# mmetcalf14/qml-cutensornet

Hardware: AMD Instinct MI355X
Metric: Gram kernel entries/sec @ 60 qubits x 6 layers (higher is better)
Workload: dtype f64 (complex128)

## Files before the change

include/qkgram.h:

```cpp
#ifndef QKGRAM_H
#define QKGRAM_H

#include <stdint.h>

#ifdef __cplusplus
extern "C" {
#endif

#define QK_OK 0
#define QK_EINVAL (-1)
#define QK_EDEVICE (-2)
#define QK_ENOMEM (-3)

#define QK_LAYOUT_LPR 0
#define QK_LAYOUT_LRP 1

#define QK_PLAN_SYMMETRIC 1u
#define QK_PLAN_QUADS 2u

#define QK_PLAN_ORIENT 4u

typedef struct qk_ctx qk_ctx;
typedef struct qk_mps_set qk_mps_set;
typedef struct qk_plan qk_plan;

typedef struct qk_stats {
  int64_t pairs;
  double flops;
  double padded_flops;
  double bytes;
  double kernel_ms;
  int32_t grid;
  int32_t max_bond;
  int32_t kernel;
  int32_t precision;
  int64_t second_pairs;
  double second_flops, second_padded_flops, second_bytes;
  double second_ms;
  int32_t second_kernel;
  int32_t queues;
  double tail_frac, second_tail_frac;
  double derive_ms;
} qk_stats;

#define QK_KERNEL_NONE 0
#define QK_KERNEL_WAVE 1
#define QK_KERNEL_SMALL 2
#define QK_KERNEL_FUSED1 3
#define QK_KERNEL_FUSED2 4
#define QK_KERNEL_RING 5
#define QK_KERNEL_LAB 6
#define QK_KERNEL_WAVE2 7
#define QK_KERNEL_WAVE2_PLAIN 9
#define QK_KERNEL_FUSED_DUAL 8
#define QK_KERNEL_FUSED_DUAL_DET 10
#define QK_KERNEL_FUSED2_DET 11
#define QK_KERNEL_FUSED1_DET 12
const char* qk_kernel_name(int32_t kernel, int32_t precision);

const char* qk_last_error(void);

int qk_device_count(void);

int qk_ctx_create(int device_id, qk_ctx** out);
int qk_ctx_destroy(qk_ctx* ctx);
int qk_ctx_set_stream(qk_ctx* ctx, void* hip_stream);
int qk_ctx_use_own_stream(qk_ctx* ctx);
int qk_ctx_synchronize(qk_ctx* ctx);
int qk_ctx_trim(qk_ctx* ctx);

int qk_mps_set_create(qk_ctx* ctx, int32_t n_states, int32_t n_sites, const int32_t* bond_dims,
                      const double* const* site_tensors, int32_t layout, qk_mps_set** out);
int qk_mps_set_destroy(qk_mps_set* set);
int qk_mps_set_info(const qk_mps_set* set, int32_t* n_states, int32_t* n_sites, int32_t* max_padded_bond,
                    int64_t* device_bytes);

int qk_mps_set_image(const qk_mps_set* set, int64_t* n_doubles, const double** planes_dev, int32_t* dims_true, int64_t* offsets);
int qk_mps_set_copy_image(const qk_mps_set* set, double* dst, int64_t n_doubles);
int qk_mps_set_from_packed(qk_ctx* ctx, int32_t n_states, int32_t n_sites, const int32_t* dims_true, const int64_t* offsets,
                           const double* planes_dev, int64_t n_doubles, qk_mps_set** out);

int qk_mps_set_precision(const qk_mps_set* set);
int qk_mps_set_to_f32(qk_ctx* ctx, const qk_mps_set* src, qk_mps_set** out);

int64_t qk_pack_state_size(int32_t n_sites, const int32_t* bond_dims);
int qk_pack_state(int32_t n_sites, const int32_t* bond_dims, const double* const* site_tensors, int32_t layout,
                  double* out, int64_t* site_offsets );

int qk_plan_create(int32_t n_sites, int32_t nx, const int32_t* x_dims, int32_t ny, const int32_t* y_dims,
                   uint32_t flags, int32_t world_size, int32_t rank, int32_t block, qk_plan** out);
int qk_plan_destroy(qk_plan* plan);
int64_t qk_plan_num_pairs(const qk_plan* plan);
int64_t qk_plan_total_pairs(const qk_plan* plan);
int64_t qk_plan_max_pairs_per_rank(const qk_plan* plan);
const int32_t* qk_plan_pairs(const qk_plan* plan);
int qk_plan_stats(const qk_plan* plan, qk_stats* out);
int64_t qk_plan_first_run(const qk_plan* plan);
int qk_plan_queues(const qk_plan* plan, int64_t* qstart );
int32_t qk_plan_edge_sites(const qk_plan* plan);
int qk_plan_create_all(int32_t n_sites, int32_t nx, const int32_t* x_dims, int32_t ny, const int32_t* y_dims,
                       uint32_t flags, int32_t world_size, qk_plan** out);
int qk_plan_cost(const qk_plan* plan, double* plan_ms, int32_t* threads, double* tile_reuse_bytes);

int qk_gram_values(qk_ctx* ctx, const qk_mps_set* xset, const qk_mps_set* yset, const qk_plan* plan,
                   double* values_dev, double* z_dev);

int qk_gram_values_host(qk_ctx* ctx, const qk_mps_set* xset, const qk_mps_set* yset, const qk_plan* plan,
                        double* values_host, double* z_host);

int qk_scatter(qk_ctx* ctx, const int32_t* pairs_dev, const double* values_dev, int64_t n, double* k_dev,
               int64_t ld, int32_t mirror);

int qk_gram_host(qk_ctx* ctx, const qk_mps_set* xset, const qk_mps_set* yset, double* out, int64_t ld);

int qk_overlaps_host(qk_ctx* ctx, const qk_mps_set* xset, const qk_mps_set* yset, double* out);

int qk_get_stats(qk_ctx* ctx, qk_stats* out);

int qk_local_paulis_host(qk_ctx* ctx, const qk_mps_set* set, double* out ,
                         double* norms );

int qk_projected_gram_host(qk_ctx* ctx, int32_t n_sites, int32_t nx, const double* fx ,
                           int32_t ny, const double* fy , double g, double* out, int64_t ld);

int qk_local_pair_paulis_host(qk_ctx* ctx, const qk_mps_set* set, double* out2 ,
// ... 172 lines not shown
```

lab/qk_quad.h:

```cpp
#pragma once

__device__ __forceinline__ int qkq_qinv(const int d) {
  static constexpr int T[17] = {0, 1048576, 524288, 349526, 262144, 209716, 174763, 149797, 131072, 116509, 104858, 95326, 87382, 80660, 74899, 69906, 65536};
  return T[d];
}

struct QkqUnit {
  bool mine, a1, b1;
  int ta, tb, p;
};

template <bool A1, bool B1, typename XPtr>
__device__ __forceinline__ void qkq_p1(QkfTile (&T)[2][2], v2d (&fr)[4], v2d (&fs)[4], const bool primed, QkfStream cur, XPtr xp, unsigned x0, unsigned x1, const int nks,
                                       const QkfStream n0, const unsigned n1off) {
  v4d P[2][2][3];
  v2d fx[4], fy[4];
  if (!primed) qkf_load4(fr, cur);
  if (B1) {
#pragma unroll
    for (int i = 0; i < 4; ++i) fs[i] = qkf_ldg(cur.base + i * cur.step, cur.off + TILE);
  }
#pragma unroll
  for (int i = 0; i < 4; ++i) {
    fx[i] = qkf_ldx(xp + i * QKF_XSTEP, x0);
// ... 91 lines not shown
      if (FULL || i < kmax) {
        const double sp = fs[i].x + fs[i].y, sm = fs[i].x - fs[i].y;
        p1 = __builtin_amdgcn_mfma_f64_16x16x4f64(S[1][0][i], fs[i].x, p1, 0, 0, 0);
        p2 = __builtin_amdgcn_mfma_f64_16x16x4f64(T[1][0].re[i], sp, p2, 0, 0, 0);
        p3 = __builtin_amdgcn_mfma_f64_16x16x4f64(T[1][0].im[i], sm, p3, 0, 0, 0);
        if (B1) {
          r1 = __builtin_amdgcn_mfma_f64_16x16x4f64(S[1][1][i], fs[i].x, r1, 0, 0, 0);
          r2 = __builtin_amdgcn_mfma_f64_16x16x4f64(T[1][1].re[i], sp, r2, 0, 0, 0);
          r3 = __builtin_amdgcn_mfma_f64_16x16x4f64(T[1][1].im[i], sm, r3, 0, 0, 0);
        }
      }
      if (!LAST) fs[i] = qkf_ldg(i == 0 ? b0 : i == 1 ? b1 : i == 2 ? b2 : b3, o1);
      __builtin_amdgcn_sched_barrier(0);
    }
  }
  QKF_PRIO_HI();
  {
    const v4d re = p1 - p3, im = p1 - p2;
#pragma unroll
    for (int r = 0; r < 4; ++r) {
      __hip_atomic_fetch_add(d + r * rs, re[r], __ATOMIC_RELAXED, __HIP_MEMORY_SCOPE_WORKGROUP);
      __hip_atomic_fetch_add(d + r * rs + 1, im[r], __ATOMIC_RELAXED, __HIP_MEMORY_SCOPE_WORKGROUP);
    }
  }
  if (B1) {
    const v4d re = r1 - r3, im = r1 - r2;
#pragma unroll
    for (int r = 0; r < 4; ++r) {
      __hip_atomic_fetch_add(d1 + r * rs, re[r], __ATOMIC_RELAXED, __HIP_MEMORY_SCOPE_WORKGROUP);
      __hip_atomic_fetch_add(d1 + r * rs + 1, im[r], __ATOMIC_RELAXED, __HIP_MEMORY_SCOPE_WORKGROUP);
    }
  }
}

template <bool FULL, bool A1, bool B1>
__device__ __forceinline__ void qkq_p2(const QkfTile (&T)[2][2], v2d (&fr)[4], v2d (&fs)[4], const QkfStream cur, const unsigned a1off, const int ps, const int nn, const int kmax, lds_v2d* xo,
                                       const int q, const int j, const QkfStream nxt) {
  lds_double* d = (lds_double*)(xo + q * TILE + j);
  lds_double* d1 = d + 2 * QKF_XBLOCK;
  constexpr long rs = 2 * QKF_XSTEP;
  v4d S[2][2];
#pragma unroll
  for (int u = 0; u < 2; ++u)
#pragma unroll
    for (int v = 0; v < 2; ++v) S[u][v] = ((u == 0 || A1) && (v == 0 || B1)) ? T[u][v].re + T[u][v].im : (v4d){0, 0, 0, 0};
  const v2d *const c0 = cur.base, *const c1 = cur.base + cur.step, *const c2 = cur.base + 2 * cur.step, *const c3 = cur.base + 3 * cur.step;
  unsigned o0 = cur.off, o1 = cur.off + a1off;
#pragma unroll 1
  for (int tn = 0; tn + 1 < nn; ++tn) {
    o0 += TILE, o1 += TILE;
    qkq_p2_block<FULL, A1, B1, false>(T, S, fr, fs, kmax, c0, c1, c2, c3, o0, o1, d, d1, rs);
    d += 2 * ps, d1 += 2 * ps;
  }
  qkq_p2_block<FULL, A1, B1, true>(T, S, fr, fs, kmax, nxt.base, nxt.base + nxt.step, nxt.base + 2 * nxt.step, nxt.base + 3 * nxt.step, nxt.off, 0u, d, d1, rs);
}

template <int NW, int XCAP, int WPS>
__global__ __launch_bounds__(64 * NW, WPS) void qk_sweep_fused_quad_kernel(const SweepArgs g) {
  constexpr int NT = 64 * NW;
  extern __shared__ __attribute__((aligned(16))) double lds_raw[];
  lds_v2d* const XL = (lds_v2d*)lds_raw;
  long long* const slot = reinterpret_cast<long long*>(lds_raw + 2 * XCAP);
  const v2d* const xdata = reinterpret_cast<const v2d*>(g.xdata);
  const v2d* const ydata = reinterpret_cast<const v2d*>(g.ydata);
  v2d* const G0 = reinterpret_cast<v2d*>(g.scratch) + (long long)blockIdx.x * 2 * g.x_plane;
  const int tid = threadIdx.x, lane = tid & 63;
  const int wave = __builtin_amdgcn_readfirstlane(tid >> 6);
  const int j = lane & 15, q = lane >> 4;
  const int ns = g.n_sites;
  __attribute__((address_space(3))) double* const zacc = (__attribute__((address_space(3))) double*)(slot + 2);
  lds_v4i* const rec = (lds_v4i*)(slot + 2 + 32);
  long long* const m_off = reinterpret_cast<long long*>(slot + 2 + 32) + 6 * (long long)ns;
  auto rfl = [&](const int v) __attribute__((always_inline)) { return __builtin_amdgcn_readfirstlane(v); };
  auto ldl = [&](const long long* p_) __attribute__((always_inline)) {
    const long long v = *p_;
    const unsigned lo = __builtin_amdgcn_readfirstlane((unsigned)v);
    const unsigned hi = __builtin_amdgcn_readfirstlane((unsigned)((unsigned long long)v >> 32));
    return (long long)(((unsigned long long)hi << 32) | lo);
  };
  auto site = [&](const int k) __attribute__((always_inline)) {
    const v4i r0 = rec[3 * k], r1 = rec[3 * k + 1], r2 = rec[3 * k + 2];
    QkfSite s;
    s.a = rfl(r0.x), s.a2 = rfl(r0.y), s.b = rfl(r0.z), s.b2 = rfl(r0.w);
    s.at = rfl(r1.x), s.nks = rfl(r1.y), s.W = rfl(r1.z), s.small = rfl(r1.w) != 0;
    s.inv = rfl(r2.x);
    s.ps = rfl(r2.y), s.pd = 1 << s.ps, s.next = rfl(r2.z);
    s.mt = s.a / TILE, s.nt = s.b2 / TILE, s.nn = s.a2 / TILE;
    s.Ak = xdata + ldl(m_off + 2 * k);
    s.Bk = ydata + ldl(m_off + 2 * k + 1);
    return s;
  };
  struct Pieces {
    int qa_f, qb_f, ra, rb, nA, kq, n2a, nB, nC, nD, L, qinv;
  };
  auto pieces_of = [&](const QkfSite& s, const int w) __attribute__((always_inline)) {
    Pieces pc;
    pc.qa_f = s.mt >> 1, pc.qb_f = w >> 1, pc.ra = s.mt & 1, pc.rb = w & 1;
    pc.nA = s.pd * pc.qa_f * pc.qb_f;
#if defined(QKF_QUAD_MODE) && QKF_QUAD_MODE == 0
    pc.kq = 0;
#else
    pc.kq = pc.nA - pc.nA % NW;
#endif
    pc.n2a = 2 * (pc.nA - pc.kq);
    pc.nB = s.pd * pc.ra * pc.qb_f, pc.nC = s.pd * pc.qa_f * pc.rb, pc.nD = s.pd * pc.ra * pc.rb;
    pc.L = pc.kq + pc.n2a + pc.nB + pc.nC + pc.nD;
    pc.qinv = qkq_qinv(pc.qa_f);
    return pc;
  };
  auto unit_of = [&](const QkfSite& s, const int w, const Pieces& pc, const int r0) __attribute__((always_inline)) {
    QkqUnit un;
    const int left = pc.L - r0;
    const bool cut = 2 * left <= NW;
    const int sub = cut && wave >= left ? 1 : 0;
    int i = r0 + wave - sub * left;
    un.mine = cut ? wave < 2 * left : i < pc.L;
    un.a1 = un.b1 = false, un.ta = un.tb = un.p = 0;
    auto quad = [&](const int vq) __attribute__((always_inline)) {
      const int u = vq >> s.ps, qb = (u * pc.qinv) >> 20, qa = u - qb * pc.qa_f;
      un.p = vq & (s.pd - 1), un.ta = 2 * qa, un.tb = 2 * qb;
    };
    if (i < pc.kq) {
      quad(i), un.a1 = un.b1 = true;
    } else if ((i -= pc.kq) < pc.n2a) {
      quad(pc.kq + (i >> 1)), un.ta += i & 1, un.b1 = true;
    } else if ((i -= pc.n2a) < pc.nB) {
      un.p = i & (s.pd - 1), un.ta = s.mt - 1, un.tb = 2 * (i >> s.ps), un.b1 = true;
    } else if ((i -= pc.nB) < pc.nC) {
      un.p = i & (s.pd - 1), un.ta = 2 * (i >> s.ps), un.tb = w - 1, un.a1 = true;
    } else {
      i -= pc.nC;
      un.p = i & (s.pd - 1), un.ta = s.mt - 1, un.tb = w - 1;
    }
    if (cut) {
      if (un.b1) un.tb += sub, un.b1 = false;
      else if (un.a1) un.ta += sub, un.a1 = false;
      else un.mine = un.mine && sub == 0;
    }
    return un;
  };
  auto b_stream = [&](const QkfSite& s, const int s0, const QkqUnit& un) __attribute__((always_inline)) {
    return QkfStream{s.Bk + un.p * s.b2, (unsigned)((q * s.pd) * s.b2 + (s0 + un.tb) * TILE + j), 4 * s.pd * s.b2};
  };
  auto a_stream = [&](const QkfSite& s, const QkqUnit& un) __attribute__((always_inline)) {
    return QkfStream{s.Ak + un.p * s.a2, (unsigned)(((un.ta * TILE + q) * s.pd) * s.a2 + j), 4 * s.pd * s.a2};
  };
  const int xcc = qk_xcc_id();
  if (tid == 0) qk_tail_start(g);
  for (;;) {
    if (tid == 0) *slot = qk_pull(g, xcc);
    __syncthreads();
    const long long p = *slot;
    __syncthreads();
    if (p < 0) break;
    const int xi = g.pairs[2 * p], yj = g.pairs[2 * p + 1];
    qkf_step_table<XCAP, NT>(g, xi, yj, p, rec, m_off, tid, QkSegRule{XCAP, NW, true});
    const int ek = g.edge_k, k_hi = ns - ek;
    const bool edges = ek > 0;
    if (!edges)
      for (int e = tid; e < TILE * TILE; e += NT) XL[e] = (v2d){e == 0 ? 1.0 : 0.0, 0.0};
    __syncthreads();
    bool xg = false;
    int cur = 0, xb = 0;
    if (edges) {
      const v4i r0 = rec[3 * ek];
      const int a_e = rfl(r0.x), b_e = rfl(r0.z);
      xg = a_e * b_e > XCAP;
// ... 135 lines not shown
```

qml-cutensornet_amd/csrc/qk_fused.h:

```cpp
#pragma once
#include "qk_device.h"
#include "qk_plan.h"

#define QKF_PRIO_LO() __builtin_amdgcn_s_setprio(0)
#define QKF_PRIO_HI() __builtin_amdgcn_s_setprio(2)
typedef double v2d __attribute__((ext_vector_type(2)));
typedef __attribute__((address_space(3))) v2d lds_v2d;
static constexpr int QKF_XSTEP = 4 * TILE;
static constexpr int QKF_XBLOCK = TILE * TILE;


#ifndef QKF_LDS3M
#define QKF_LDS3M 0
#endif
#ifndef QKF_P2_PROBE
#define QKF_P2_PROBE 0
#endif
#ifndef QKF_ABL
#define QKF_ABL 0
#endif
#define QKF_STEP_BARRIER()                            \
  do {                                                \
    if (QKF_ABL & 4) asm volatile("s_waitcnt lgkmcnt(0)" ::: "memory"); \
    else qk_lds_barrier();                            \
  } while (0)
#define QKF_SUM(a, b) ((QKF_ABL & 1) ? (a) : (a) + (b))
#define QKF_DIF(a, b) ((QKF_ABL & 1) ? (b) : (a) - (b))
template <bool CONJB>
__device__ __forceinline__ void qkf_kstep(v4d& p1, v4d& p2, v4d& p3, const double ar, const double ai, const double br, const double bi) {
  const double sa = QKF_SUM(ar, ai), sb = CONJB ? QKF_DIF(br, bi) : QKF_SUM(br, bi);
  p1 = __builtin_amdgcn_mfma_f64_16x16x4f64(ar, br, p1, 0, 0, 0);
  p2 = __builtin_amdgcn_mfma_f64_16x16x4f64(ai, bi, p2, 0, 0, 0);
  p3 = __builtin_amdgcn_mfma_f64_16x16x4f64(sa, sb, p3, 0, 0, 0);
}

struct QkfTile {
  v4d re, im;
};

__device__ __forceinline__ v2d qkf_ldg(const v2d* __restrict__ base, const unsigned off) {
  return *reinterpret_cast<const v2d*>(reinterpret_cast<const char*>(base) + (size_t)(off * 16u));
}
#ifndef QKF_NT_A
#define QKF_NT_A 0
#endif
#ifndef QKF_NT_B
#define QKF_NT_B 0
#endif
__device__ __forceinline__ v2d qkf_ldg_nt(const v2d* __restrict__ base, const unsigned off) {
  return __builtin_nontemporal_load(reinterpret_cast<const v2d*>(reinterpret_cast<const char*>(base) + (size_t)(off * 16u)));
}
__device__ __forceinline__ v2d qkf_ldg_a(const v2d* __restrict__ base, const unsigned off) { return QKF_NT_A ? qkf_ldg_nt(base, off) : qkf_ldg(base, off); }
__device__ __forceinline__ v2d qkf_ldg_b(const v2d* __restrict__ base, const unsigned off) { return QKF_NT_B ? qkf_ldg_nt(base, off) : qkf_ldg(base, off); }
__device__ __forceinline__ v2d qkf_ldx(const v2d* __restrict__ base, const unsigned off) { return qkf_ldg(base, off); }
__device__ __forceinline__ v2d qkf_ldx(const lds_v2d* base, const unsigned off) { return base[off]; }

struct QkfStream {
  const v2d* base;
  unsigned off;
  int step;
  int lim = 4;
};
__device__ __forceinline__ const v2d* qkf_kbase(const v2d* const base, const int step, const int i, const int lim) { return base + max(min(i, lim - 1), 0) * step; }
__device__ __forceinline__ void qkf_load4(v2d (&fr)[4], const QkfStream& st) {
#pragma unroll
  for (int i = 0; i < 4; ++i) fr[i] = qkf_ldg(qkf_kbase(st.base, st.step, i, st.lim), st.off);
}
__device__ __forceinline__ v2d qkf_ldgb(const v2d* __restrict__ base, const unsigned boff) {
  const v2d* const at = reinterpret_cast<const v2d*>(reinterpret_cast<const char*>(base) + (size_t)boff);
  return QKF_NT_B ? __builtin_nontemporal_load(at) : *at;
}
struct QkfXLds {
  const lds_v2d* p;
  __device__ __forceinline__ void advance() { p += 4 * QKF_XSTEP; }
  __device__ __forceinline__ v2d kstep(const int i) const { return p[i * QKF_XSTEP]; }
};
struct QkfXGlobal {
  const v2d* base;
  unsigned bo;
  __device__ __forceinline__ void advance() { bo += 4 * QKF_XSTEP * 16u; }
  __device__ __forceinline__ v2d kstep(const int i) const { return *reinterpret_cast<const v2d*>(reinterpret_cast<const char*>(base + i * QKF_XSTEP) + (size_t)bo); }
};
__device__ __forceinline__ QkfXLds qkf_xcursor(const lds_v2d* xp, const unsigned xoff) { return QkfXLds{xp + xoff}; }
__device__ __forceinline__ QkfXGlobal qkf_xcursor(const v2d* xp, const unsigned xoff) { return QkfXGlobal{xp, xoff * 16u}; }

// ... 420 lines not shown
  QKF_PRIO_HI();
  t0.re = acc[0] + acc[1], t0.im = acc[2] - acc[0] + acc[1];
  if (HAS1) t1.re = acc[3] + acc[4], t1.im = acc[5] - acc[3] + acc[4];
}
__device__ __forceinline__ long long qkf_uniform(const long long v) {
  const unsigned lo = __builtin_amdgcn_readfirstlane((unsigned)v);
  const unsigned hi = __builtin_amdgcn_readfirstlane((unsigned)((unsigned long long)v >> 32));
  return (long long)(((unsigned long long)hi << 32) | lo);
}

template <int NW, bool PAIRS>
__device__ __forceinline__ QkEdgeUnit qkf_edge_unit_of(const int u, const int mt, const int nt, const int inv) {
  if constexpr (PAIRS) return qk_edge_unit(u, mt, nt, NW, inv);
  const int tb = (u * inv) >> 20;
  return QkEdgeUnit{u - tb * mt, tb, false, true};
}
template <int NW, bool PAIRS, int SETS>
__device__ __forceinline__ void qkf_edge_prefix(const SweepArgs& g, const int xi, const int yj, const int a, const int b, lds_v2d* const xl, v2d* const xg, const bool to_global, const int wave,
                                                const int q, const int j, const bool swap = false) {
  const v2d* const Lx = reinterpret_cast<const v2d*>(swap ? g.yedge : g.xedge) + qkf_uniform((swap ? g.yedge_offs : g.xedge_offs)[2 * (long long)xi]);
  const v2d* const Ly = reinterpret_cast<const v2d*>(swap ? g.xedge : g.yedge) + qkf_uniform((swap ? g.xedge_offs : g.yedge_offs)[2 * (long long)yj]);
  const int mt = a / TILE, nt = b / TILE, ng = (1 << g.edge_k) >> 4, inv = qk_recip20(mt), units = PAIRS ? qk_edge_units(mt, nt, NW) : mt * nt;
  for (int u = wave; u < units; u += NW) {
    const QkEdgeUnit un = qkf_edge_unit_of<NW, PAIRS>(u, mt, nt, inv);
    if (!un.mine) continue;
    QkfTile T0, T1;
    const unsigned oy = (unsigned)(q * b + un.tb0 * TILE + j), ox = (unsigned)(q * a + un.ta * TILE + j);
    if (un.has1) qkf_edge_unit<true, 1>(T0, T1, Ly, oy, b, Lx, ox, a, ng);
    else qkf_edge_unit<false, SETS>(T0, T1, Ly, oy, b, Lx, ox, a, ng);
    const int at = un.ta * (b * TILE) + (un.tb0 * TILE + q) * TILE + j;
    if (to_global) {
#pragma unroll
      for (int r = 0; r < 4; ++r) xg[at + r * QKF_XSTEP] = (v2d){T0.re[r], T0.im[r]};
      if (un.has1) {
#pragma unroll
        for (int r = 0; r < 4; ++r) xg[at + QKF_XBLOCK + r * QKF_XSTEP] = (v2d){T1.re[r], T1.im[r]};
      }
    } else {
#pragma unroll
      for (int r = 0; r < 4; ++r) xl[at + r * QKF_XSTEP] = (v2d){T0.re[r], T0.im[r]};
      if (un.has1) {
#pragma unroll
        for (int r = 0; r < 4; ++r) xl[at + QKF_XBLOCK + r * QKF_XSTEP] = (v2d){T1.re[r], T1.im[r]};
      }
    }
  }
}

template <int NW, bool PAIRS, int SETS>
__device__ __forceinline__ void qkf_edge_suffix(const SweepArgs& g, const int xi, const int yj, const int a, const int b, const lds_v2d* const xl, const v2d* const xg, const bool from_global,
                                                __attribute__((address_space(3))) double* zacc, const int wave, const int q, const int j, const bool swap = false) {
  const v2d* const Rx = reinterpret_cast<const v2d*>(swap ? g.yedge : g.xedge) + qkf_uniform((swap ? g.yedge_offs : g.xedge_offs)[2 * (long long)xi + 1]);
  const v2d* const Ry = reinterpret_cast<const v2d*>(swap ? g.xedge : g.yedge) + qkf_uniform((swap ? g.xedge_offs : g.yedge_offs)[2 * (long long)yj + 1]);
  const int mt = a / TILE, nt = b / TILE, ng = (1 << g.edge_k) >> 4, inv = qk_recip20(mt), units = PAIRS ? qk_edge_units(mt, nt, NW) : mt * nt;
  double zr = 0, zi = 0;
  for (int u = wave; u < units; u += NW) {
    const QkEdgeUnit un = qkf_edge_unit_of<NW, PAIRS>(u, mt, nt, inv);
    if (!un.mine) continue;
    QkfTile T0, T1;
    const unsigned oy = (unsigned)(q * b + un.tb0 * TILE + j), ox = (unsigned)(q * a + un.ta * TILE + j);
    if (un.has1) qkf_edge_unit<true, 1>(T0, T1, Ry, oy, b, Rx, ox, a, ng);
    else qkf_edge_unit<false, SETS>(T0, T1, Ry, oy, b, Rx, ox, a, ng);
    const int at = un.ta * (b * TILE) + (un.tb0 * TILE + q) * TILE + j;
#pragma unroll
    for (int r = 0; r < 4; ++r) {
      const v2d x = from_global ? xg[at + r * QKF_XSTEP] : (v2d)xl[at + r * QKF_XSTEP];
      zr += x.x * T0.re[r] - x.y * T0.im[r], zi += x.x * T0.im[r] + x.y * T0.re[r];
    }
    if (un.has1) {
#pragma unroll
      for (int r = 0; r < 4; ++r) {
        const v2d x = from_global ? xg[at + QKF_XBLOCK + r * QKF_XSTEP] : (v2d)xl[at + QKF_XBLOCK + r * QKF_XSTEP];
        zr += x.x * T1.re[r] - x.y * T1.im[r], zi += x.x * T1.im[r] + x.y * T1.re[r];
      }
    }
  }
#pragma unroll
  for (int o = 32; o > 0; o >>= 1) zr += __shfl_xor(zr, o), zi += __shfl_xor(zi, o);
  if ((q | j) == 0) zacc[2 * wave] = zr, zacc[2 * wave + 1] = zi;
}

struct QkfSite {
  int a, a2, b, b2, at, nks, mt, nt, nn, W, inv, inv2, pd, ps, next;
  bool small, sw;
  const v2d *Ak, *Bk;
};
typedef int v4i __attribute__((ext_vector_type(4)));
typedef __attribute__((address_space(3))) v4i lds_v4i;

template <int XCAP, int NT, bool ITEM_RECIPS = false>
__device__ __forceinline__ void qkf_step_table(const SweepArgs& g, const int xi, const int yj, const long long pair, lds_v4i* const rec, long long* const m_off, const int tid, const QkSegRule rule) {
  const int ns = g.n_sites, n1 = ns + 1;
  const int32_t* const xd = g.xdims + (long long)xi * n1;
  const int32_t* const yd = g.ydims + (long long)yj * n1;
  const int32_t* const xt = g.xtrue + (long long)xi * n1;
  const int32_t* const yt = g.ytrue + (long long)yj * n1;
  const v2d* const xdata = reinterpret_cast<const v2d*>(g.xdata);
  const v2d* const ydata = reinterpret_cast<const v2d*>(g.ydata);
  auto put = [&](const int e, const int len, const int o, const bool sw, const v2d* const X, const v2d* const Y) __attribute__((always_inline)) {
    const QkStepRec r = qk_step_record(xd, xt, yd, yt, e, len, o, sw, rule, ITEM_RECIPS);
    rec[3 * e] = (v4i){r.w[0], r.w[1], r.w[2], r.w[3]};
    rec[3 * e + 1] = (v4i){r.w[4], r.w[5], r.w[6], r.w[7]};
    rec[3 * e + 2] = (v4i){r.w[8], r.w[9], r.w[10], r.w[11]};
    m_off[2 * e] = (long long)(((const char*)(o ? Y : X) - (const char*)xdata) / 16);
    m_off[2 * e + 1] = (long long)(((const char*)(o ? X : Y) - (const char*)ydata) / 16);
  };
  auto plain = [&](const int e, const int o, const bool sw) __attribute__((always_inline)) {
    put(e, 1, o, sw, xdata + (g.xoffs[(long long)xi * ns + e] >> 1), ydata + (g.yoffs[(long long)yj * ns + e] >> 1));
  };
  if (g.seg == nullptr) {
    for (int e = tid; e < ns; e += NT) plain(e, 0, false);
    return;
  }
  const int ek = g.edge_k, k_hi = ns - ek;
  const unsigned long long w0 = g.seg[4 * pair], w1 = g.seg[4 * pair + 1], o0 = g.seg[4 * pair + 2], o1 = g.seg[4 * pair + 3];
  for (int e = ek + tid; e < k_hi; e += NT) {
    const int i = e - ek;
    const bool merged = qk_seg_bit(w0, w1, i) && e + 1 < k_hi;
    const int len = merged ? 2 : 1, o = qk_seg_bit(o0, o1, i) ? 1 : 0;
    const bool sw = qk_seg_bit(o0, o1, i + len) != (o != 0);
    if (merged)
      put(e, 2, o, sw, reinterpret_cast<const v2d*>(g.xmg) + (g.xmg_offs[(long long)xi * g.merge_steps + i] >> 1),
          reinterpret_cast<const v2d*>(g.ymg) + (g.ymg_offs[(long long)yj * g.merge_steps + i] >> 1));
    else plain(e, o, sw);
  }
}

#ifdef QKF_PROF
#define QKF_PROF_DECL() \
  unsigned long long pf[8] = {0, 0, 0, 0, 0, 0, 0, 0}, pt = __builtin_amdgcn_s_memtime(); \
  const unsigned long long pt0 = pt
#define QKF_STAMP(i)                                              \
  do {                                                            \
    const unsigned long long now_ = __builtin_amdgcn_s_memtime(); \
    pf[i] += now_ - pt;                                           \
    pt = now_;                                                    \
  } while (0)
#define QKF_PROF_FLUSH()                                             \
  do {                                                               \
    if (lane == 0) {                                                 \
      pf[7] = __builtin_amdgcn_s_memtime() - pt0;                    \
      for (int i_ = 0; i_ < 8; ++i_) atomicAdd(g.prof + i_, pf[i_]); \
    }                                                                \
  } while (0)
#else
#define QKF_PROF_DECL()
#define QKF_STAMP(i)
#define QKF_PROF_FLUSH()
#endif

#define QKF_PULLER(NT) ((NT) - 64)
__device__ __forceinline__ void qkf_pull_next(const SweepArgs& g, const int xcc, int& gang_round, long long* const word) {
  const long long pp = qk_pull(g, xcc);
  qk_gang_sync(g, xcc, pp >= 0, gang_round);
  *word = pp;
}

template <int NW, int S, int XCAP, int WPS, bool DET = false>
__global__ __launch_bounds__(64 * NW, WPS) void qk_sweep_fused_kernel(const SweepArgs g) {
  constexpr int NT = 64 * NW;
  extern __shared__ __attribute__((aligned(16))) double lds_raw[];
  lds_v2d* const XL = (lds_v2d*)lds_raw;
  long long* const slot = reinterpret_cast<long long*>(lds_raw + 2 * XCAP);
  const v2d* const xdata = reinterpret_cast<const v2d*>(g.xdata);
  const v2d* const ydata = reinterpret_cast<const v2d*>(g.ydata);
  v2d* const G0 = reinterpret_cast<v2d*>(g.scratch) + (long long)blockIdx.x * 2 * g.x_plane;
  const int tid = threadIdx.x, lane = tid & 63;
  const int wave = __builtin_amdgcn_readfirstlane(tid >> 6);
  const int j = lane & 15, q = lane >> 4;
  const int ns = g.n_sites;
  __attribute__((address_space(3))) double* const zacc = (__attribute__((address_space(3))) double*)(slot + 2);
  lds_v4i* const rec = (lds_v4i*)(slot + 2 + 32);
  long long* const m_off = reinterpret_cast<long long*>(slot + 2 + 32) + 6 * (long long)ns;
  lds_int* const tbroken = (lds_int*)(m_off + 2 * (long long)ns);
  lds_int* const turn0 = tbroken + 2;
  auto rfl = [&](const int v) __attribute__((always_inline)) { return __builtin_amdgcn_readfirstlane(v); };
  auto ldl = [&](const long long* p_) __attribute__((always_inline)) {
    const long long v = *p_;
    const unsigned lo = __builtin_amdgcn_readfirstlane((unsigned)v);
    const unsigned hi = __builtin_amdgcn_readfirstlane((unsigned)((unsigned long long)v >> 32));
    return (long long)(((unsigned long long)hi << 32) | lo);
  };
  auto site = [&](const int k) __attribute__((always_inline)) {
    const v4i r0 = rec[3 * k], r1 = rec[3 * k + 1], r2 = rec[3 * k + 2];
    QkfSite s;
    s.a = rfl(r0.x), s.a2 = rfl(r0.y), s.b = rfl(r0.z), s.b2 = rfl(r0.w);
    s.at = rfl(r1.x), s.nks = rfl(r1.y), s.W = rfl(r1.z), s.small = (rfl(r1.w) & QK_REC_SMALL) != 0, s.sw = (rfl(r1.w) & QK_REC_SWITCH) != 0;
    s.inv = rfl(r2.x), s.inv2 = rfl(r2.w);
    s.ps = rfl(r2.y), s.pd = 1 << s.ps, s.next = rfl(r2.z);
    s.mt = s.a / TILE, s.nt = s.b2 / TILE, s.nn = s.a2 / TILE;
    s.Ak = xdata + ldl(m_off + 2 * k);
    s.Bk = ydata + ldl(m_off + 2 * k + 1);
    return s;
  };
  auto item_of = [&](const QkfSite& s, const int w, const int it) __attribute__((always_inline)) {
    return DET ? qk_unit_decode_ordered(it, s.ps, s.mt, s.inv) : qk_unit_decode(it, s.mt, w, s.inv, qk_unit_recip_of(s.inv2, w == s.W));
  };
  auto b_stream = [&](const QkfSite& s, const int s0, const int w, const int it) __attribute__((always_inline)) {
    const QkUnit un = item_of(s, w, it);
    return QkfStream{s.Bk + un.p * s.b2, (unsigned)((q * s.pd) * s.b2 + (s0 + un.tc) * TILE + j), 4 * s.pd * s.b2, min(4, s.nks)};
  };
  auto a_stream = [&](const QkfSite& s, const int w, const int it) __attribute__((always_inline)) {
    const QkUnit un = item_of(s, w, it);
    return QkfStream{s.Ak + un.p * s.a2, (unsigned)(((un.ta * TILE + q) * s.pd) * s.a2 + j), 4 * s.pd * s.a2, min(4, (s.at - un.ta * TILE + 3) >> 2)};
  };
  QKF_PROF_DECL();
  const int xcc = qk_xcc_id();
  int gang_round = 0;
  if (tid == 0) qk_tail_start(g);
  for (;;) {
    if (tid == 0) {
      const long long pp_ = qk_pull(g, xcc);
      qk_gang_sync(g, xcc, pp_ >= 0, gang_round);
      *slot = pp_;
    }
    __syncthreads();
    const long long p = *slot;
    __syncthreads();
    if (p < 0) break;
    const int xi = g.pairs[2 * p], yj = g.pairs[2 * p + 1];
    qkf_step_table<XCAP, NT, true>(g, xi, yj, p, rec, m_off, tid, QkSegRule{XCAP, NW * S, false});
    const int ek = g.edge_k, k_hi = ns - ek;
    const bool edges = ek > 0;
    if (!edges)
      for (int e = tid; e < TILE * TILE; e += NT) XL[e] = (v2d){e == 0 ? 1.0 : 0.0, 0.0};
    if constexpr (DET)
      for (int e = tid; e < 2 * g.turn_ints + 2; e += NT) tbroken[e] = 0;
    int tsel = 0;
    __syncthreads();
    bool xg = false;
    int cur = 0, xb = 0;
    if (edges) {
      const v4i r0 = rec[3 * ek];
      const int a_e = rfl(r0.x), b_e = rfl(r0.z);
      const bool o1 = !DET && (rfl(rec[3 * ek + 1].w) & QK_REC_ORIENT) != 0;
      xg = a_e * b_e > XCAP;
      qkf_edge_prefix<NW, QKF_EDGE_PAIRS(WPS), QKF_EDGE_SETS(WPS)>(g, o1 ? yj : xi, o1 ? xi : yj, a_e, b_e, XL, G0, xg, wave, q, j, o1);
      __syncthreads();
    }
    QKF_STAMP(0);
    QkfTile T[S];
    v2d fr[4];
    bool primed = false;
    QkfSite sn = site(ek);
    for (int k = ek; k < k_hi;) {
      const QkfSite sc = sn;
      k = sc.next;
      if (k < k_hi) sn = site(k);
      const int a = sc.a, a2 = sc.a2, b = sc.b, mt = sc.mt, nt = sc.nt, W = sc.W;
      const bool small = sc.small;
      v2d* const Gc = G0 + (long long)cur * g.x_plane;
      v2d* const Gn = G0 + (long long)(cur ^ 1) * g.x_plane;
      if (small && xg) {
        for (int e = tid; e < a * b; e += NT) XL[e] = Gc[e];
        __syncthreads();
        xg = false, xb = 0;
      } else if (!small && !xg) {
        for (int e = tid; e < a * b; e += NT) Gc[e] = XL[xb + e];
        __syncthreads();
        xg = true;
      }
      const int n_out = sc.b2 * a2;
      const bool pingpong = small && a * b + n_out <= XCAP;
      const int ob = !small ? 0 : pingpong ? (xb == 0 ? XCAP - n_out : 0) : 0;
      if (pingpong && !DET)
        for (int e = tid; e < n_out; e += NT) XL[ob + e] = (v2d){0.0, 0.0};
      QKF_STAMP(1);
      for (int s0 = 0; s0 < nt; s0 += W) {
        const int w = min(W, nt - s0), items = sc.pd * mt * w;
        lds_int* const tcur = turn0 + tsel * g.turn_ints;
        if constexpr (DET) {
          for (int e = tid; e < g.turn_ints; e += NT) turn0[(tsel ^ 1) * g.turn_ints + e] = 0;
        } else if (!small) {
          for (int e = tid; e < w * TILE * a2; e += NT) XL[e] = (v2d){0.0, 0.0};
          QKF_STEP_BARRIER();
        }
        QKF_STAMP(6);
        for (int r0 = 0; r0 < items; r0 += NW * S) {
          const int L = min(S, (items - r0 + NW - 1) / NW);
          const bool multi = L > 1;
          const int it0 = r0 + wave;
          auto phase1 = [&](auto xbase) __attribute__((always_inline)) {
#pragma unroll 1
            for (int s = 0; s < L; ++s) {
              if (multi) qkf_rotate<S>(T, L);
              const int it = it0 + NW * s;
              if (it < items) {
                const int ta = item_of(sc, w, it).ta;
                const bool more = s + 1 < L && it + NW < items;
                const QkfStream nxt = more ? b_stream(sc, s0, w, it + NW) : a_stream(sc, w, it0);
                qkf_p1_tile(T[S - 1], fr, primed, b_stream(sc, s0, w, it), xbase, (unsigned)(ta * (b * TILE) + q * TILE + j), sc.nks, nxt);
                primed = true;
              }
            }
          };
          if (xg) phase1((const v2d*)Gc);
          else phase1((const lds_v2d*)(XL + xb));
          QKF_STAMP(2);
          if (small && r0 == 0 && !(DET && pingpong)) {
            QKF_STEP_BARRIER();
            if (!pingpong && !DET) {
              for (int e = tid; e < n_out; e += NT) XL[e] = (v2d){0.0, 0.0};
              QKF_STEP_BARRIER();
            }
          }
          QKF_STAMP(3);
          const bool last_round = s0 + W >= nt && r0 + NW * S >= items;
#pragma unroll 1
          for (int s = 0; s < S; ++s) {
            const int it = it0 + NW * s;
            if (it >= items) break;
            if (multi) qkf_rotate<S>(T, L);
            const QkUnit un = item_of(sc, w, it);
            const int ta = un.ta, tbl = un.tc;
            const int kmax = min(4, (sc.at - ta * TILE + 3) >> 2);
            const bool more = s + 1 < S && it + NW < items;
            const int wn = min(sn.W, sn.nt);
            const bool chain = !more && last_round && k < k_hi && wave < sn.pd * sn.mt * wn;
            const QkfStream nxt = more ? a_stream(sc, w, it + NW) : chain ? b_stream(sn, 0, wn, wave) : a_stream(sc, w, it);
            const int tix = sc.pd * ta + un.p;
            const QkfTurn turn{tcur + tbl * sc.nn, tix, tbroken, g.err};
            constexpr int FORM = DET ? 0 : WPS >= 4 ? QKF_P2_FORM_TWO : QKF_P2_FORM_ONE;
            if (!DET && sc.sw) {
              lds_double* const dsw = (lds_double*)(XL + ob + tbl * (a2 * TILE) + q * TILE + j);
              if (FORM != 0 && kmax == 4) qkf_p2_switch<true, false, FORM>(T[S - 1], T[S - 1], fr, primed, a_stream(sc, w, it), 4, sc.nn, 4, dsw, 0, nxt);
              else qkf_p2_switch<false, false, FORM>(T[S - 1], T[S - 1], fr, primed, a_stream(sc, w, it), kmax, sc.nn, kmax, dsw, 0, nxt);
            } else if (kmax == 4) qkf_p2_item<true, DET, FORM>(T[S - 1], fr, primed, a_stream(sc, w, it), w * QKF_XBLOCK, sc.nn, 4, XL + ob + tbl * QKF_XBLOCK, q, j, nxt, turn);
            else qkf_p2_item<false, DET, FORM>(T[S - 1], fr, primed, a_stream(sc, w, it), w * QKF_XBLOCK, sc.nn, kmax, XL + ob + tbl * QKF_XBLOCK, q, j, nxt, turn);
            primed = more || chain;
          }
          QKF_STAMP(4);
        }
        QKF_STEP_BARRIER();
        tsel ^= 1;
        QKF_STAMP(5);
        if (!small && nt > W) {
          for (int tn = 0; tn < sc.nn; ++tn)
            for (int e = tid; e < w * QKF_XBLOCK; e += NT) Gn[(long long)tn * (sc.b2 * TILE) + s0 * QKF_XBLOCK + e] = XL[tn * w * QKF_XBLOCK + e];
          __syncthreads();
          QKF_STAMP(1);
        }
      }
      if (!small) {
        if (nt > W) cur ^= 1;
        else xg = false, xb = 0;
      } else {
        xb = ob;
      }
    }
    const int fl_end = DET ? 0 : rfl(rec[3 * (k_hi - 1) + 1].w);
    const bool sw_end = (fl_end & QK_REC_SWITCH) != 0, o_end = ((fl_end & QK_REC_ORIENT) != 0) != sw_end;
    if (edges) {
      const v4i r0 = rec[3 * (k_hi - 1)];
      const int a_l = rfl(r0.y), b_l = rfl(r0.w), a_e = sw_end ? b_l : a_l, b_e = sw_end ? a_l : b_l;
      qkf_edge_suffix<NW, QKF_EDGE_PAIRS(WPS), QKF_EDGE_SETS(WPS)>(g, o_end ? yj : xi, o_end ? xi : yj, a_e, b_e, (const lds_v2d*)(XL + xb), (const v2d*)(G0 + (long long)cur * g.x_plane), xg, zacc, wave,
                                                                   q, j, o_end);
      __syncthreads();
    }
    if (tid == 0) {
      v2d zz = {0.0, 0.0};
      if (edges)
        for (int w_ = 0; w_ < NW; ++w_) zz.x += zacc[2 * w_], zz.y += zacc[2 * w_ + 1];
      else zz = xg ? G0[(long long)cur * g.x_plane] : (v2d)XL[xb];
      if (o_end) zz.y = -zz.y;
      g.values[p] = zz.x * zz.x + zz.y * zz.y;
      if (g.z) {
        g.z[2 * p] = zz.x;
        g.z[2 * p + 1] = zz.y;
      }
    }
    __syncthreads();
  }
  if (tid == 0) qk_tail_exit(g);
  QKF_PROF_FLUSH();
}

template <bool HAS1, typename XPtr>
__device__ __forceinline__ void qkf_p1_dual(QkfTile& t0, QkfTile& t1, v2d (&fr)[4], v2d (&fs)[4], const bool primed, QkfStream cur, XPtr xp, unsigned xoff, const int nks,
                                            const QkfStream nxt) {
  v4d p1 = {0, 0, 0, 0}, p2 = {0, 0, 0, 0}, p3 = {0, 0, 0, 0}, r1 = {0, 0, 0, 0}, r2 = {0, 0, 0, 0}, r3 = {0, 0, 0, 0};
  v2d fx[4];
  if (!primed) qkf_load4(fr, cur);
  if (HAS1) {
#pragma unroll
    for (int i = 0; i < 4; ++i) fs[i] = qkf_ldg(cur.base + i * cur.step, cur.off + TILE);
  }
#pragma unroll
  for (int i = 0; i < 4; ++i) fx[i] = qkf_ldx(xp + i * QKF_XSTEP, xoff);
  const int ng = (nks + 3) >> 2, last = nks - 4 * (ng - 1);
  QKF_PRIO_LO();
  int gq = 0;
  if (ng >= 2) {
    gq = 1;
    cur.off += 4 * cur.step, xoff += 4 * QKF_XSTEP;
#pragma unroll
    for (int i = 0; i < 4; ++i) {
      if (i == 0) {
        const v4d z = {0, 0, 0, 0};
        const double sa = QKF_SUM(fx[0].x, fx[0].y);
        p1 = __builtin_amdgcn_mfma_f64_16x16x4f64(fx[0].x, fr[0].x, z, 0, 0, 0);
        p2 = __builtin_amdgcn_mfma_f64_16x16x4f64(fx[0].y, fr[0].y, z, 0, 0, 0);
        p3 = __builtin_amdgcn_mfma_f64_16x16x4f64(sa, QKF_SUM(fr[0].x, fr[0].y), z, 0, 0, 0);
        if (HAS1) {
          r1 = __builtin_amdgcn_mfma_f64_16x16x4f64(fx[0].x, fs[0].x, z, 0, 0, 0);
          r2 = __builtin_amdgcn_mfma_f64_16x16x4f64(fx[0].y, fs[0].y, z, 0, 0, 0);
          r3 = __builtin_amdgcn_mfma_f64_16x16x4f64(sa, QKF_SUM(fs[0].x, fs[0].y), z, 0, 0, 0);
        }
      } else {
        qkf_kstep<false>(p1, p2, p3, fx[i].x, fx[i].y, fr[i].x, fr[i].y);
        if (HAS1) qkf_kstep<false>(r1, r2, r3, fx[i].x, fx[i].y, fs[i].x, fs[i].y);
      }
      if (!(QKF_ABL & 2)) fr[i] = qkf_ldg_b(cur.base + i * cur.step, cur.off);
      if (HAS1 && !(QKF_ABL & 2)) fs[i] = qkf_ldg_b(cur.base + i * cur.step, cur.off + TILE);
      if (!(QKF_ABL & 8)) fx[i] = qkf_ldx(xp + i * QKF_XSTEP, xoff);
      __builtin_amdgcn_sched_barrier(0);
    }
  }
#pragma unroll 1
  for (; gq + 1 < ng; ++gq) {
    cur.off += 4 * cur.step, xoff += 4 * QKF_XSTEP;
#pragma unroll
    for (int i = 0; i < 4; ++i) {
      qkf_kstep<false>(p1, p2, p3, fx[i].x, fx[i].y, fr[i].x, fr[i].y);
      if (HAS1) qkf_kstep<false>(r1, r2, r3, fx[i].x, fx[i].y, fs[i].x, fs[i].y);
      if (!(QKF_ABL & 2)) fr[i] = qkf_ldg_b(cur.base + i * cur.step, cur.off);
      if (HAS1 && !(QKF_ABL & 2)) fs[i] = qkf_ldg_b(cur.base + i * cur.step, cur.off + TILE);
      if (!(QKF_ABL & 8)) fx[i] = qkf_ldx(xp + i * QKF_XSTEP, xoff);
      __builtin_amdgcn_sched_barrier(0);
    }
  }
#pragma unroll
  for (int i = 0; i < 4; ++i) {
    if (i < last) {
      qkf_kstep<false>(p1, p2, p3, fx[i].x, fx[i].y, fr[i].x, fr[i].y);
      if (HAS1) qkf_kstep<false>(r1, r2, r3, fx[i].x, fx[i].y, fs[i].x, fs[i].y);
    }
    if (!(QKF_ABL & 2)) fr[i] = qkf_ldg(nxt.base + i * nxt.step, nxt.off);
    __builtin_amdgcn_sched_barrier(0);
  }
  QKF_PRIO_HI();
  t0.re = p1 - p2, t0.im = p3 - p1 - p2;
  if (HAS1) t1.re = r1 - r2, t1.im = r3 - r1 - r2;
}

template <bool FULL, bool HAS1>
__device__ __forceinline__ void qkf_p2_block(const QkfTile& t0, const QkfTile& t1, const v4d& s0, const v4d& s1, v2d (&fr)[4], const int kmax, const v2d* const b0, const v2d* const b1,
// ... 33 lines not shown
  if (HAS1) {
#pragma unroll
    for (int r = 0; r < 4; ++r) {
      __hip_atomic_fetch_add(d1 + r * rs, re1[r], __ATOMIC_RELAXED, __HIP_MEMORY_SCOPE_WORKGROUP);
      __hip_atomic_fetch_add(d1 + r * rs + 1, im1[r], __ATOMIC_RELAXED, __HIP_MEMORY_SCOPE_WORKGROUP);
    }
  }
}
template <bool FULL, bool HAS1, bool DET>
__device__ __forceinline__ void qkf_p2_dual_turn(const QkfTile& t0, const QkfTile& t1, v2d (&fr)[4], v2d (&fs)[4], QkfStream cur, const int ps, const int nn, const int kmax, lds_v2d* xo, const int q,
                                            const int j, const QkfStream nxt, const bool nxt_p1, const unsigned n1, const QkfTurn turn = QkfTurn{nullptr, 0, nullptr, nullptr}) {
  __attribute__((address_space(3))) double* d = (__attribute__((address_space(3))) double*)(xo + q * TILE + j);
#pragma unroll 1
  for (int tn = 0; tn < nn; ++tn) {
    v4d p1 = {0, 0, 0, 0}, p2 = {0, 0, 0, 0}, p3 = {0, 0, 0, 0}, r1 = {0, 0, 0, 0}, r2 = {0, 0, 0, 0}, r3 = {0, 0, 0, 0};
    const bool fin = tn + 1 == nn;
    const v2d* const rb = fin ? nxt.base : cur.base;
    const int rs = fin ? nxt.step : cur.step;
    cur.off = fin ? nxt.off : cur.off + TILE;
    QKF_PRIO_LO();
#pragma unroll
    for (int i = 0; i < 4; ++i) {
      if (FULL || i < kmax) {
        qkf_kstep<true>(p1, p2, p3, t0.re[i], t0.im[i], fr[i].x, fr[i].y);
        if (HAS1) qkf_kstep<true>(r1, r2, r3, t1.re[i], t1.im[i], fr[i].x, fr[i].y);
      }
      fr[i] = qkf_ldg_a(rb + i * rs, cur.off);
      __builtin_amdgcn_sched_barrier(0);
    }
    QKF_PRIO_HI();
    {
      const v4d re = p1 + p2, im = p3 - p1 + p2;
      if constexpr (DET) qkf_turn_add(d, (long)2 * QKF_XSTEP, re, im, turn, tn);
      else {
#pragma unroll
        for (int r = 0; r < 4; ++r) {
          __hip_atomic_fetch_add(d + r * 2 * QKF_XSTEP, re[r], __ATOMIC_RELAXED, __HIP_MEMORY_SCOPE_WORKGROUP);
          __hip_atomic_fetch_add(d + r * 2 * QKF_XSTEP + 1, im[r], __ATOMIC_RELAXED, __HIP_MEMORY_SCOPE_WORKGROUP);
        }
      }
    }
    if (HAS1) {
      const v4d re = r1 + r2, im = r3 - r1 + r2;
      __attribute__((address_space(3))) double* const d1 = d + 2 * QKF_XBLOCK;
      if constexpr (DET) qkf_turn_add(d1, (long)2 * QKF_XSTEP, re, im, QkfTurn{turn.at + nn, turn.idx, turn.broken, turn.gerr}, tn);
      else {
#pragma unroll
        for (int r = 0; r < 4; ++r) {
          __hip_atomic_fetch_add(d1 + r * 2 * QKF_XSTEP, re[r], __ATOMIC_RELAXED, __HIP_MEMORY_SCOPE_WORKGROUP);
          __hip_atomic_fetch_add(d1 + r * 2 * QKF_XSTEP + 1, im[r], __ATOMIC_RELAXED, __HIP_MEMORY_SCOPE_WORKGROUP);
        }
      }
    }
    d += 2 * ps;
  }
}

template <bool FULL, bool HAS1, bool DET = false>
__device__ __forceinline__ void qkf_p2_dual(const QkfTile& t0, const QkfTile& t1, v2d (&fr)[4], v2d (&fs)[4], QkfStream cur, const int ps, const int nn, const int kmax, lds_v2d* xo, const int q,
                                            const int j, const QkfStream nxt, const bool nxt_p1, const unsigned n1, const QkfTurn turn = QkfTurn{nullptr, 0, nullptr, nullptr}) {
  if constexpr (DET) {
    qkf_p2_dual_turn<FULL, HAS1, DET>(t0, t1, fr, fs, cur, ps, nn, kmax, xo, q, j, nxt, nxt_p1, n1, turn);
    return;
  }
  lds_double* d = (lds_double*)(xo + q * TILE + j);
  lds_double* d1 = d + 2 * QKF_XBLOCK;
  if constexpr (QKF_P2_FORM_DUAL != 0) {
    qkf_p2_blocks<FULL, HAS1, false>(t0, t1, fr, cur, 4, nxt, nn, kmax, d, 2 * QKF_XBLOCK, 2 * ps);
    return;
  }
  constexpr long rs = 2 * QKF_XSTEP;
  const v4d s0 = t0.re + t0.im, s1 = HAS1 ? t1.re + t1.im : s0;
  const v2d *const c0 = cur.base, *const c1 = cur.base + cur.step, *const c2 = cur.base + 2 * cur.step, *const c3 = cur.base + 3 * cur.step;
  unsigned off = cur.off;
#pragma unroll 1
  for (int tn = 0; tn + 1 < nn; ++tn) {
    off += TILE;
    qkf_p2_block<FULL, HAS1>(t0, t1, s0, s1, fr, kmax, c0, c1, c2, c3, off, d, d1, rs);
    d += 2 * ps, d1 += 2 * ps;
  }
  qkf_p2_block<FULL, HAS1>(t0, t1, s0, s1, fr, kmax, nxt.base, nxt.base + nxt.step, nxt.base + 2 * nxt.step, nxt.base + 3 * nxt.step, nxt.off, d, d1, rs);
}

template <int NW, int XCAP, int WPS, bool DET = false>
__global__ __launch_bounds__(64 * NW, WPS) void qk_sweep_fused_dual_kernel(const SweepArgs g) {
  constexpr int NT = 64 * NW;
  extern __shared__ __attribute__((aligned(16))) double lds_raw[];
  lds_v2d* const XL = (lds_v2d*)lds_raw;
  long long* const slot = reinterpret_cast<long long*>(lds_raw + 2 * XCAP);
  const v2d* const xdata = reinterpret_cast<const v2d*>(g.xdata);
  const v2d* const ydata = reinterpret_cast<const v2d*>(g.ydata);
  v2d* const G0 = reinterpret_cast<v2d*>(g.scratch) + (long long)blockIdx.x * 2 * g.x_plane;
  const int tid = threadIdx.x, lane = tid & 63;
  const int wave = __builtin_amdgcn_readfirstlane(tid >> 6);
  const int j = lane & 15, q = lane >> 4;
  const int ns = g.n_sites;
  __attribute__((address_space(3))) double* const zacc = (__attribute__((address_space(3))) double*)(slot + 2);
  lds_v4i* const rec = (lds_v4i*)(slot + 2 + 32);
  long long* const m_off = reinterpret_cast<long long*>(slot + 2 + 32) + 6 * (long long)ns;
  lds_int* const tbroken = (lds_int*)(m_off + 2 * (long long)ns);
  lds_int* const turn0 = tbroken + 2;
  auto rfl = [&](const int v) __attribute__((always_inline)) { return __builtin_amdgcn_readfirstlane(v); };
  auto ldl = [&](const long long* p_) __attribute__((always_inline)) {
    const long long v = *p_;
    const unsigned lo = __builtin_amdgcn_readfirstlane((unsigned)v);
    const unsigned hi = __builtin_amdgcn_readfirstlane((unsigned)((unsigned long long)v >> 32));
    return (long long)(((unsigned long long)hi << 32) | lo);
  };
  auto site = [&](const int k) __attribute__((always_inline)) {
    const v4i r0 = rec[3 * k], r1 = rec[3 * k + 1], r2 = rec[3 * k + 2];
    QkfSite s;
    s.a = rfl(r0.x), s.a2 = rfl(r0.y), s.b = rfl(r0.z), s.b2 = rfl(r0.w);
    s.at = rfl(r1.x), s.nks = rfl(r1.y), s.W = rfl(r1.z), s.small = (rfl(r1.w) & QK_REC_SMALL) != 0, s.sw = (rfl(r1.w) & QK_REC_SWITCH) != 0;
    s.inv = rfl(r2.x);
    s.ps = rfl(r2.y), s.pd = 1 << s.ps, s.next = rfl(r2.z);
    s.mt = s.a / TILE, s.nt = s.b2 / TILE, s.nn = s.a2 / TILE;
    s.Ak = xdata + ldl(m_off + 2 * k);
    s.Bk = ydata + ldl(m_off + 2 * k + 1);
    return s;
  };
  auto pair_of = [&](const QkfSite& s, const int v) __attribute__((always_inline)) { return qk_unit_decode_ordered(v, s.ps, s.mt, s.inv); };
  auto b_stream = [&](const QkfSite& s, const int s0, const int v, const int half) __attribute__((always_inline)) {
    const QkUnit un = pair_of(s, v);
    return QkfStream{s.Bk + un.p * s.b2, (unsigned)((q * s.pd) * s.b2 + (s0 + 2 * un.tc + half) * TILE + j), 4 * s.pd * s.b2};
  };
  struct Unit {
    bool mine, has1;
    int v, half;
  };
  auto unit_of = [&](const QkfSite& s, const int w, const int units, const int r0) __attribute__((always_inline)) {
    Unit un;
    const int left = units - r0;
    const bool halves = 2 * left <= NW;
    un.half = (halves && wave >= left) ? 1 : 0;
    un.v = r0 + wave - (un.half ? left : 0);
    const int tp = pair_of(s, un.v).tc;
    const bool second = 2 * tp + 1 < w;
    un.mine = un.v < units && (un.half == 0 || second);
    un.has1 = !halves && second;
    return un;
  };
  auto a_stream = [&](const QkfSite& s, const int v) __attribute__((always_inline)) {
    const QkUnit un = pair_of(s, v);
    return QkfStream{s.Ak + un.p * s.a2, (unsigned)(((un.ta * TILE + q) * s.pd) * s.a2 + j), 4 * s.pd * s.a2};
  };
  QKF_PROF_DECL();
  const int xcc = qk_xcc_id();
  int gang_round = 0;
  if (tid == 0) qk_tail_start(g);
  if (tid == QKF_PULLER(NT)) qkf_pull_next(g, xcc, gang_round, slot);
  __syncthreads();
  long long p = slot[0];
  int psel = 0;
  auto table_of = [&](const long long pp) __attribute__((always_inline)) {
    if (pp < 0) return;
    const int xi_ = g.pairs[2 * pp], yj_ = g.pairs[2 * pp + 1];
    qkf_step_table<XCAP, NT>(g, xi_, yj_, pp, rec, m_off, tid, QkSegRule{XCAP, NW, true});
  };
  table_of(p);
  while (p >= 0) {
    const int xi = g.pairs[2 * p], yj = g.pairs[2 * p + 1];
    const int ek = g.edge_k, k_hi = ns - ek;
    const bool edges = ek > 0;
    if (!edges)
      for (int e = tid; e < TILE * TILE; e += NT) XL[e] = (v2d){e == 0 ? 1.0 : 0.0, 0.0};
    if constexpr (DET)
      for (int e = tid; e < 2 * g.turn_ints + 2; e += NT) tbroken[e] = 0;
    int tsel = 0;
    __syncthreads();
    bool xg = false;
    int cur = 0, xb = 0;
    if (edges) {
      const v4i r0 = rec[3 * ek];
      const int a_e = rfl(r0.x), b_e = rfl(r0.z);
      const bool o1 = !DET && (rfl(rec[3 * ek + 1].w) & QK_REC_ORIENT) != 0;
      xg = a_e * b_e > XCAP;
      qkf_edge_prefix<NW, QKF_EDGE_PAIRS(WPS), QKF_EDGE_SETS(WPS)>(g, o1 ? yj : xi, o1 ? xi : yj, a_e, b_e, XL, G0, xg, wave, q, j, o1);
      __syncthreads();
    }
    QKF_STAMP(0);
    QkfTile T0, T1;
    v2d fr[4], fs[4];
    bool primed = false;
    QkfSite sn = site(ek);
    for (int k = ek; k < k_hi;) {
      const QkfSite sc = sn;
      k = sc.next;
      if (k < k_hi) sn = site(k);
      const int a = sc.a, a2 = sc.a2, b = sc.b, mt = sc.mt, nt = sc.nt, W = sc.W;
      const bool small = sc.small;
      v2d* const Gc = G0 + (long long)cur * g.x_plane;
      v2d* const Gn = G0 + (long long)(cur ^ 1) * g.x_plane;
      if (small && xg) {
        for (int e = tid; e < a * b; e += NT) XL[e] = Gc[e];
        __syncthreads();
        xg = false, xb = 0;
      } else if (!small && !xg) {
        for (int e = tid; e < a * b; e += NT) Gc[e] = XL[xb + e];
        __syncthreads();
        xg = true;
      }
      const int n_out = sc.b2 * a2;
      const bool pingpong = small && a * b + n_out <= XCAP;
      const int ob = !small ? 0 : pingpong ? (xb == 0 ? XCAP - n_out : 0) : 0;
      if (pingpong && !DET)
        for (int e = tid; e < n_out; e += NT) XL[ob + e] = (v2d){0.0, 0.0};
      QKF_STAMP(1);
      for (int s0 = 0; s0 < nt; s0 += W) {
        const int w = min(W, nt - s0), units = sc.pd * mt * ((w + 1) >> 1);
        lds_int* const tcur = turn0 + tsel * g.turn_ints;
        if constexpr (DET) {
          for (int e = tid; e < g.turn_ints; e += NT) turn0[(tsel ^ 1) * g.turn_ints + e] = 0;
        } else if (!small) {
          for (int e = tid; e < w * TILE * a2; e += NT) XL[e] = (v2d){0.0, 0.0};
          QKF_STEP_BARRIER();
        }
        for (int r0 = 0; r0 < units; r0 += NW) {
          const Unit un = unit_of(sc, w, units, r0);
          const int v = un.v;
          const bool mine = un.mine, has1 = un.has1;
          const QkUnit pr = pair_of(sc, v);
          const int tp = pr.tc, ta = pr.ta;
          if (mine) {
            const QkfStream bs = b_stream(sc, s0, v, un.half), as = a_stream(sc, v);
            const unsigned xoff = (unsigned)(ta * (b * TILE) + q * TILE + j);
            if (xg) {
              if (has1) qkf_p1_dual<true>(T0, T1, fr, fs, primed, bs, (const v2d*)Gc, xoff, sc.nks, as);
              else qkf_p1_dual<false>(T0, T1, fr, fs, primed, bs, (const v2d*)Gc, xoff, sc.nks, as);
            } else {
              if (has1) qkf_p1_dual<true>(T0, T1, fr, fs, primed, bs, (const lds_v2d*)(XL + xb), xoff, sc.nks, as);
              else qkf_p1_dual<false>(T0, T1, fr, fs, primed, bs, (const lds_v2d*)(XL + xb), xoff, sc.nks, as);
            }
          }
          QKF_STAMP(2);
          if (small && r0 == 0 && !(DET && pingpong)) {
            QKF_STEP_BARRIER();
            if (!pingpong && !DET) {
              for (int e = tid; e < n_out; e += NT) XL[e] = (v2d){0.0, 0.0};
              QKF_STEP_BARRIER();
            }
          }
          QKF_STAMP(3);
          if (mine) {
            const int kmax = min(4, (sc.at - ta * TILE + 3) >> 2);
            QkfStream nxt = a_stream(sc, v);
            bool np1 = false;
            if (r0 + NW < units) {
              const Unit nu = unit_of(sc, w, units, r0 + NW);
              if (nu.mine) nxt = b_stream(sc, s0, nu.v, nu.half), np1 = true;
            } else if (s0 + W < nt) {
              const int w2 = min(W, nt - s0 - W);
              const Unit nu = unit_of(sc, w2, sc.pd * mt * ((w2 + 1) >> 1), 0);
              if (nu.mine) nxt = b_stream(sc, s0 + W, nu.v, nu.half), np1 = true;
            } else if (k < k_hi) {
              const int w2 = min(sn.W, sn.nt);
              const Unit nu = unit_of(sn, w2, sn.pd * sn.mt * ((w2 + 1) >> 1), 0);
              if (nu.mine) nxt = b_stream(sn, 0, nu.v, nu.half), np1 = true;
            }
            const unsigned nd1 = 0;
            lds_v2d* const xo = XL + ob + (2 * tp + un.half) * QKF_XBLOCK;
            const QkfTurn tp_turn{tcur + (2 * tp + un.half) * sc.nn, sc.pd * ta + pr.p, tbroken, g.err};
            if (!DET && sc.sw) {
              lds_double* const dsw = (lds_double*)(XL + ob + (2 * tp + un.half) * (a2 * TILE) + q * TILE + j);
              constexpr int FORM = QKF_P2_FORM_DUAL;
              if (FORM != 0 && kmax == 4) {
                if (has1) qkf_p2_switch<true, true, FORM>(T0, T1, fr, true, a_stream(sc, v), 4, sc.nn, 4, dsw, 2 * a2 * TILE, nxt);
                else qkf_p2_switch<true, false, FORM>(T0, T1, fr, true, a_stream(sc, v), 4, sc.nn, 4, dsw, 0, nxt);
              } else {
                if (has1) qkf_p2_switch<false, true, FORM>(T0, T1, fr, true, a_stream(sc, v), 4, sc.nn, kmax, dsw, 2 * a2 * TILE, nxt);
                else qkf_p2_switch<false, false, FORM>(T0, T1, fr, true, a_stream(sc, v), 4, sc.nn, kmax, dsw, 0, nxt);
              }
            } else if (has1) {
              if (kmax == 4) qkf_p2_dual<true, true, DET>(T0, T1, fr, fs, a_stream(sc, v), w * QKF_XBLOCK, sc.nn, 4, xo, q, j, nxt, np1, nd1, tp_turn);
              else qkf_p2_dual<false, true, DET>(T0, T1, fr, fs, a_stream(sc, v), w * QKF_XBLOCK, sc.nn, kmax, xo, q, j, nxt, np1, nd1, tp_turn);
            } else {
              if (kmax == 4) qkf_p2_dual<true, false, DET>(T0, T1, fr, fs, a_stream(sc, v), w * QKF_XBLOCK, sc.nn, 4, xo, q, j, nxt, np1, nd1, tp_turn);
              else qkf_p2_dual<false, false, DET>(T0, T1, fr, fs, a_stream(sc, v), w * QKF_XBLOCK, sc.nn, kmax, xo, q, j, nxt, np1, nd1, tp_turn);
            }
            primed = np1;
          }
          QKF_STAMP(4);
        }
        QKF_STEP_BARRIER();
        tsel ^= 1;
        QKF_STAMP(5);
        if (!small && nt > W) {
          for (int tn = 0; tn < sc.nn; ++tn)
            for (int e = tid; e < w * QKF_XBLOCK; e += NT) Gn[(long long)tn * (sc.b2 * TILE) + s0 * QKF_XBLOCK + e] = XL[tn * w * QKF_XBLOCK + e];
          __syncthreads();
        }
      }
      if (!small) {
        if (nt > W) cur ^= 1;
        else xg = false, xb = 0;
      } else {
        xb = ob;
      }
    }
    if (tid == QKF_PULLER(NT)) qkf_pull_next(g, xcc, gang_round, slot + (psel ^ 1));
    const int fl_end = DET ? 0 : rfl(rec[3 * (k_hi - 1) + 1].w);
    const bool sw_end = (fl_end & QK_REC_SWITCH) != 0, o_end = ((fl_end & QK_REC_ORIENT) != 0) != sw_end;
    if (edges) {
      const v4i r0 = rec[3 * (k_hi - 1)];
      const int a_l = rfl(r0.y), b_l = rfl(r0.w), a_e = sw_end ? b_l : a_l, b_e = sw_end ? a_l : b_l;
      qkf_edge_suffix<NW, QKF_EDGE_PAIRS(WPS), QKF_EDGE_SETS(WPS)>(g, o_end ? yj : xi, o_end ? xi : yj, a_e, b_e, (const lds_v2d*)(XL + xb), (const v2d*)(G0 + (long long)cur * g.x_plane), xg, zacc, wave,
                                                                   q, j, o_end);
    }
    __syncthreads();
    const long long pn = slot[psel ^ 1];
    if (tid == 0) {
      v2d zz = {0.0, 0.0};
      if (edges)
        for (int w_ = 0; w_ < NW; ++w_) zz.x += zacc[2 * w_], zz.y += zacc[2 * w_ + 1];
      else zz = xg ? G0[(long long)cur * g.x_plane] : (v2d)XL[xb];
      if (o_end) zz.y = -zz.y;
      g.values[p] = zz.x * zz.x + zz.y * zz.y;
      if (g.z) {
        g.z[2 * p] = zz.x;
        g.z[2 * p + 1] = zz.y;
      }
    }
    table_of(pn);
    if (!edges) __syncthreads();
    p = pn, psel ^= 1;
    QKF_STAMP(6);
  }
  if (tid == 0) qk_tail_exit(g);
  QKF_PROF_FLUSH();
}

template <typename T>
__global__ void qk_interleave_kernel(const T* __restrict__ src, T* __restrict__ dst, const int32_t* __restrict__ dims, const int64_t* __restrict__ offs,
                                     const int n_sites, const long long n_tensors) {
  typedef T v2 __attribute__((ext_vector_type(2)));
  for (long long t = blockIdx.x; t < n_tensors; t += gridDim.x) {
    const long long s = t / n_sites;
    const int k = (int)(t - s * n_sites);
    const long long plane = (long long)dims[s * (n_sites + 1) + k] * 2 * dims[s * (n_sites + 1) + k + 1];
    const T* re = src + offs[t];
    const T* im = re + plane;
    v2* d = reinterpret_cast<v2*>(dst + offs[t]);
    for (long long e = threadIdx.x; e < plane; e += blockDim.x) d[e] = (v2){re[e], im[e]};
  }
}

template <int N>
__device__ __forceinline__ void qkw_wait_vmcnt() {
  static_assert(N >= 0 && N < 64, "vmcnt is a 6-bit field");
  asm volatile("s_waitcnt vmcnt(%0)" ::"n"(N) : "memory");
}

template <int NG, typename SRC>
__global__ __launch_bounds__(64, 2) void qk_sweep_wave2_kernel(const SweepArgs g) {
  constexpr bool F32 = sizeof(SRC) == 4;
  static_assert(!F32 || NG > 0, "complex64 images go through the LDS ring");
  constexpr int ES = F32 ? 8 : 16;
  constexpr int GROUP = F32 ? 128 : 256;
  __shared__ long long slot;
  __shared__ v2d ring[NG > 0 ? NG * GROUP : 1];
  typedef __attribute__((address_space(3))) void* lds_ptr_t;
  const int lane = threadIdx.x, j = lane & 15, q = lane >> 4;
  const unsigned ring_lds = (unsigned)(uintptr_t)(lds_ptr_t)ring + (F32 ? (unsigned)(q * 128 + j * 8) : (unsigned)lane * 16u);
  const int ns = g.n_sites, n1 = ns + 1;
  const char* const xdata = reinterpret_cast<const char*>(g.xdata);
  const char* const ydata = reinterpret_cast<const char*>(g.ydata);
  auto uni = [](const int v) __attribute__((always_inline)) { return __builtin_amdgcn_readfirstlane(v); };
  auto unil = [](const long long v) __attribute__((always_inline)) {
    const unsigned lo = __builtin_amdgcn_readfirstlane((unsigned)v);
    const unsigned hi = __builtin_amdgcn_readfirstlane((unsigned)((unsigned long long)v >> 32));
    return (long long)(((unsigned long long)hi << 32) | lo);
  };
  const int xcc = qk_xcc_id();
  if (lane == 0) qk_tail_start(g);
  for (;;) {
    if (lane == 0) slot = qk_pull(g, xcc);
    __syncthreads();
    const long long p = unil(slot);
    __syncthreads();
    if (p < 0) break;
    typedef const __attribute__((address_space(4))) int* sint_p;
    typedef const __attribute__((address_space(4))) int64_t* slong_p;
    const int xi = ((sint_p)g.pairs)[2 * p], yj = ((sint_p)g.pairs)[2 * p + 1];
    const sint_p xd = (sint_p)(g.xdims + (long long)xi * n1);
    const sint_p yd = (sint_p)(g.ydims + (long long)yj * n1);
    const sint_p xt = (sint_p)(g.xtrue + (long long)xi * n1);
    const sint_p yt = (sint_p)(g.ytrue + (long long)yj * n1);
    const slong_p xo = (slong_p)(g.xoffs + (long long)xi * ns);
    const slong_p yo = (slong_p)(g.yoffs + (long long)yj * ns);
    QkfTile XA[2][2], XN[2][2];
#pragma unroll
    for (int u = 0; u < 2; ++u)
#pragma unroll
      for (int v = 0; v < 2; ++v) XA[u][v].re = XA[u][v].im = XN[u][v].re = XN[u][v].im = (v4d){0, 0, 0, 0};
    XA[0][0].re[0] = (lane == 0) ? 1.0 : 0.0;
    int f_k = 0, f_i = 0, f_n = 0, f_slot = 0, c_slot = 0;
    int f_a2 = 0, f_b2 = 0;
    const char* f_A = xdata;
// ... 155 lines not shown
```

qml-cutensornet_amd/csrc/qk_plan.h:

```cpp
#pragma once
#include "../../include/qkgram.h"

#include <algorithm>
#include <cstdint>
#include <cstdio>
#include <vector>

int qk_fail(int code, const char* fmt, ...) __attribute__((format(printf, 2, 3)));

#ifndef QKF_XCAP_ONE_V
#define QKF_XCAP_ONE_V 8192
#endif
#ifndef QKF_XCAP_TWO_V
#define QKF_XCAP_TWO_V 4608
#endif
#ifndef QKF_TWO_WGS
#define QKF_TWO_WGS 2
#endif
static constexpr int QKF_XCAP_ONE = QKF_XCAP_ONE_V, QKF_XCAP_TWO = QKF_XCAP_TWO_V;
static constexpr int QK_TILE = 16;
static inline int qk_pad16(int x) { return (x + QK_TILE - 1) / QK_TILE * QK_TILE; }
static constexpr int GMAX = 4;

#if defined(__HIPCC__)
#define QK_HD __host__ __device__
#else
#define QK_HD
#endif
struct QkUnit {
  int ta, tc, p;
};
QK_HD static inline int qk_unit_cols(const int w, const bool dual) { return dual ? (w + 1) >> 1 : w; }
QK_HD static inline int qk_recip20(const int d) { return ((1 << 20) + d - 1) / d; }
QK_HD static inline int qk_recip15(const int d) { return ((1 << 15) + d - 1) / d; }
QK_HD static inline int qk_unit_recips(const int nt, const int W, const bool dual) {
  const int wl = nt - (nt - 1) / W * W;
  return qk_recip15(qk_unit_cols(W, dual)) | (qk_recip15(qk_unit_cols(wl, dual)) << 16);
}
QK_HD static inline int qk_unit_recip_of(const int recips, const bool full_strip) { return full_strip ? (recips & 0xffff) : (int)((unsigned)recips >> 16); }
QK_HD static inline QkUnit qk_unit_decode(const int v, const int mt, const int wc, const int inv_mt, const int inv_wc) {
  const int c = (v * inv_mt) >> 20, p = (c * inv_wc) >> 15;
  return QkUnit{v - c * mt, c - p * wc, p};
}
QK_HD static inline QkUnit qk_unit_decode_ordered(const int v, const int ps, const int mt, const int inv_mt) {
  const int u = v >> ps, tc = (u * inv_mt) >> 20;
  return QkUnit{u - tc * mt, tc, v & ((1 << ps) - 1)};
}

struct QkEdgeUnit {
  int ta, tb0;
  bool has1, mine;
};
QK_HD static inline int qk_edge_units(const int mt, const int nt, const int NW) {
  const int pairs = mt * ((nt + 1) >> 1), r0 = (pairs - 1) / NW * NW, left = pairs - r0;
  return 2 * left <= NW ? r0 + 2 * left : pairs;
}
QK_HD static inline QkEdgeUnit qk_edge_unit(const int u, const int mt, const int nt, const int NW, const int inv_mt) {
  const int pairs = mt * ((nt + 1) >> 1), r0 = (pairs - 1) / NW * NW, left = pairs - r0;
  const bool halves = 2 * left <= NW, single = halves && u >= r0, half = halves && u >= r0 + left;
  const int v = u - (half ? left : 0), tp = (v * inv_mt) >> 20;
  const bool second = 2 * tp + 1 < nt;
  return QkEdgeUnit{v - tp * mt, 2 * tp + (half ? 1 : 0), !single && second, u < (halves ? r0 + 2 * left : pairs) && (!half || second)};
}

static constexpr int QK_STEP_PRICE = 375;
static constexpr int QK_SEG_BITS = 128;
struct QkSegRule {
  int xcap, cap;
  bool dual;
};
struct QkSegMask {
  unsigned long long w[2];
};
QK_HD static inline bool qk_seg_bit(const unsigned long long w0, const unsigned long long w1, const int i) { return i < QK_SEG_BITS && (((i < 64 ? w0 : w1) >> (i & 63)) & 1ull) != 0; }
QK_HD static inline bool qk_seg_one_round(const QkSegRule& r, const int pmt, const int nt) { return pmt * (r.dual ? (nt + 1) / 2 : nt) <= r.cap; }
QK_HD static inline bool qk_seg_small(const QkSegRule& r, const int a, const int a2, const int b, const int b2, const int pd) {
  return a * b <= r.xcap && a2 * b2 <= r.xcap && (qk_seg_one_round(r, pd * (a / QK_TILE), b2 / QK_TILE) || a * b + a2 * b2 <= r.xcap);
}
QK_HD static inline long long qk_step_instr(const int pd, const int a, const int a2, const int b, const int b2, const int at, const int bt) {
  return 3ll * pd * (b2 / QK_TILE) * ((long long)(a / QK_TILE) * ((bt + 3) >> 2) + (long long)(a2 / QK_TILE) * ((at + 3) >> 2));
}
QK_HD static inline bool qk_merge_admissible(const QkSegRule& r, const int32_t* const xd, const int32_t* const yd, const int e) {
  const int a = xd[e], am = xd[e + 1], a2 = xd[e + 2], b = yd[e], bm = yd[e + 1], b2 = yd[e + 2];
  const long long work_m = 4ll * a * b2 * (b + a2), work_p = 2ll * a * bm * (b + am) + 2ll * am * b2 * (bm + a2);
  return (qk_seg_small(r, a, a2, b, b2, 4) || (!qk_seg_small(r, a, am, b, bm, 2) && !qk_seg_small(r, am, a2, bm, b2, 2))) && work_m <= work_p;
}
static constexpr int QK_SWITCH_PRICE = 40;
QK_HD static inline bool qk_seg_small_o(const QkSegRule& r, const int o, const int a, const int a2, const int b, const int b2, const int pd) {
  return o ? qk_seg_small(r, b, b2, a, a2, pd) : qk_seg_small(r, a, a2, b, b2, pd);
}
QK_HD static inline QkSegMask qk_segment_chain(const int32_t* const xd, const int32_t* const xt, const int32_t* const yd, const int32_t* const yt, const int n_sites, const int ek,
                                               const QkSegRule& rule, const int parities, const bool greedy, long long* const objective = nullptr, int* const steps = nullptr,
                                               const int assoc = 0, const int switch_price = QK_SWITCH_PRICE, QkSegMask* const orient = nullptr, int* const switches = nullptr) {
  const int m = n_sites - 2 * ek;
  const int mode = (greedy || m + 1 > QK_SEG_BITS) ? 0 : assoc;
  auto may = [&](const int i, const int o) {
    return i + 1 < m && i < QK_SEG_BITS && ((parities >> (i & 1)) & 1) != 0 && qk_merge_admissible(rule, o ? yd : xd, o ? xd : yd, ek + i);
  };
  auto step_cost = [&](const int i, const int o, const int len) {
    const int e = ek + i;
    return (o ? qk_step_instr(2 * len, yd[e], yd[e + len], xd[e], xd[e + len], yt[e], xt[e]) : qk_step_instr(2 * len, xd[e], xd[e + len], yd[e], yd[e + len], xt[e], yt[e])) + QK_STEP_PRICE;
  };
  auto may_switch = [&](const int i, const int o, const int len) {
    const int e = ek + i;
    return qk_seg_small_o(rule, o, xd[e], xd[e + len], yd[e], yd[e + len], 2 * len);
  };
  auto bit = [](const QkSegMask& k, const int i) { return qk_seg_bit(k.w[0], k.w[1], i); };
  auto set = [](QkSegMask& k, const int i) { k.w[i >> 6] |= 1ull << (i & 63); };
  QkSegMask take[2] = {{{0ull, 0ull}}, {{0ull, 0ull}}};
  QkSegMask swit[2] = {{{0ull, 0ull}}, {{0ull, 0ull}}};
  int o_start = 0;
  if (greedy) {
    for (int i = 0; i < m && i < QK_SEG_BITS; ++i)
      if (may(i, 0)) set(take[0], i);
  } else if (mode <= 1) {
    struct Best {
      long long c;
      int sw, n1, st;
    };
    auto less = [](const Best& a, const Best& b) { return a.c != b.c ? a.c < b.c : a.sw != b.sw ? a.sw < b.sw : a.n1 != b.n1 ? a.n1 < b.n1 : a.st < b.st; };
    auto same = [](const Best& a, const Best& b) { return a.c == b.c && a.sw == b.sw && a.n1 == b.n1 && a.st == b.st; };
    Best f1[2] = {{0, 0, 0, 0}, {0, 0, 0, 0}}, f2[2] = {{0, 0, 0, 0}, {0, 0, 0, 0}};
    const int no = mode == 1 ? 2 : 1;
    for (int i = m - 1; i >= 0; --i) {
      Best f0[2] = {{0, 0, 0, 0}, {0, 0, 0, 0}};
      for (int o = 0; o < no; ++o) {
        auto cand = [&](const int len, bool& sw) {
          const Best* const rest = len == 2 ? f2 : f1;
          const long long c = step_cost(i, o, len);
          Best b{c + rest[o].c, rest[o].sw, rest[o].n1 + o, rest[o].st + 1};
          sw = false;
          if (mode == 1 && may_switch(i, o, len)) {
            const Best s{c + switch_price + rest[1 - o].c, rest[1 - o].sw + 1, rest[1 - o].n1 + o, rest[1 - o].st + 1};
            if (less(s, b)) b = s, sw = true;
          }
          return b;
        };
        bool sw = false, swm = false;
        Best b = cand(1, sw);
        if (may(i, o)) {
          const Best bm = cand(2, swm);
          if (less(bm, b) || (same(bm, b) && (i & 1) == 0)) b = bm, sw = swm, set(take[o], i);
        }
        if (sw) set(swit[o], i);
        f0[o] = b;
      }
      for (int o = 0; o < 2; ++o) f2[o] = f1[o], f1[o] = f0[o];
    }
    if (mode == 1 && less(f1[1], f1[0])) o_start = 1;
  } else {
    o_start = mode == 3 ? 1 : 0;
  }
  QkSegMask out{{0ull, 0ull}}, ori{{0ull, 0ull}};
  long long obj = 0;
  int n_steps = 0, n_sw = 0, o = o_start;
  for (int i = 0; i < m; ++n_steps) {
    const bool mg = mode >= 2 ? may(i, o) : bit(take[o], i);
    const int len = mg ? 2 : 1;
    const bool sw = mode >= 2 ? may_switch(i, o, len) : bit(swit[o], i);
    if (mg) set(out, i);
    if (o)
      for (int s = i; s < i + len; ++s) set(ori, s);
    obj += step_cost(i, o, len) + (sw ? switch_price : 0);
    if (sw) o ^= 1, ++n_sw;
    i += len;
  }
  if (o) set(ori, m);
  if (objective) *objective = obj;
  if (steps) *steps = n_steps;
  if (orient) *orient = ori;
  if (switches) *switches = n_sw;
  return out;
}

struct QkStepRec {
  int w[12];
};
static constexpr int QK_REC_SMALL = 1, QK_REC_ORIENT = 2, QK_REC_SWITCH = 4;
QK_HD static inline QkStepRec qk_step_record(const int32_t* xd, const int32_t* xt, const int32_t* yd, const int32_t* yt, const int e, const int len, const int o, const bool sw,
                                             const QkSegRule& rule, const bool item_recips) {
  if (o) {
    const int32_t* t = xd;
    xd = yd, yd = t, t = xt, xt = yt, yt = t;
  }
  const int a = xd[e], a2 = xd[e + len], b = yd[e], b2 = yd[e + len];
  const bool small = qk_seg_small(rule, a, a2, b, b2, 2 * len);
  const int mt = a / QK_TILE, nt = b2 / QK_TILE;
  const int lim = rule.xcap / (QK_TILE * a2), W = small ? nt : (lim < 1 ? 1 : lim < nt ? lim : nt);
  return QkStepRec{{a, a2, b, b2, xt[e], (yt[e] + 3) >> 2, W, (small ? QK_REC_SMALL : 0) | (o ? QK_REC_ORIENT : 0) | (sw ? QK_REC_SWITCH : 0), qk_recip20(mt), len == 2 ? 2 : 1, e + len,
                    item_recips ? qk_unit_recips(nt, W, false) : 0}};
}

struct qk_ctx;

struct qk_plan {
  int n_sites = 0, nx = 0, ny = 0;
  bool symmetric = false;
  bool quad = false;
  int world = 1, rank = 0;
  int64_t total_pairs = 0, max_per_rank = 0;
  std::vector<int32_t> pairs;
  std::vector<int32_t> groups;
  int group = 1;
  qk_stats stats{};
  qk_stats second{};
  int64_t n_first = 0;
  int nq = 1;
  int64_t qstart[17] = {0};
  int edge_k = 0;
  bool second_wave2 = false;
  double fit_two = 1.0;
  double fit_narrow = 1.0;
  double tile_reuse_bytes = 0;
  double plan_ms = 0;
  int plan_threads = 1;
  qk_ctx* up_ctx = nullptr;
  int32_t* d_pairs = nullptr;
  int32_t* d_groups = nullptr;
  unsigned long long* d_seg = nullptr;
  unsigned long long seg_key[8] = {0};
};

struct QkSweepPolicy {
  int variant = 20;
  int wgs_per_cu = 2;
  bool wave_path = true;
  bool wave2_ring = true;
  bool wave2_path = true;
  bool small_path = true;
  int fused_path = 1;
  int fused_split = 1;
  int fused_wgs = 0;
  bool deterministic = false;
  int merge_mode = 2;
  int assoc_mode = 1;
  int switch_price = QK_SWITCH_PRICE;
  bool fused_dual = true;
  bool gang = false;
};

struct QkSetShape {
  int max_pad = 0, precision = 64, n_sites = 0;
};

struct QkSweepRun {
  int kernel = QK_KERNEL_NONE;
  long long grid = 0;
  size_t lds = 0;
  long long first = 0, count = 0;
  int nq = 1, gang_n = 0;
  bool gang2 = false;
};

struct QkSweepChoice {
  int rc = QK_OK;
  char err[192] = {};
  int n_runs = 0;
  QkSweepRun run[2];
  long long launched_grid = 0;
  long long x_plane = 0, t_plane = 0;
  int turn_ints = 0;
  size_t scratch_bytes = 0;
  bool interleaved = false;
  bool fused_images = false;
  int queues = 1;
  bool tails = false;
};

static inline QkSweepChoice qk_choose_sweep(const QkSweepPolicy& p, const qk_plan& plan, const QkSetShape& x, const QkSetShape& y, const int num_cus) {
  QkSweepChoice ch;
  const long long np = (long long)plan.pairs.size() / 2;
  const bool f32 = x.precision == 32, quad = plan.quad, det = p.deterministic;
  const int n = x.n_sites, max_pad = std::max(x.max_pad, y.max_pad);
  const bool grouped = p.variant == 14 && !f32 && !quad, duo = p.variant == 16 && !f32 && !quad;
  const long long chains = quad ? 4 : (duo ? 2 : 1);
  const long long units = quad ? np / 4 : grouped ? (long long)plan.groups.size() / 2 : (duo ? (np + 1) / 2 : np);
  ch.x_plane = (grouped ? GMAX : 1) * (long long)x.max_pad * y.max_pad, ch.t_plane = 2 * ch.x_plane;
  ch.turn_ints = det ? (y.max_pad / QK_TILE) * (x.max_pad / QK_TILE) : 0;
  const size_t lds_meta = 16 + 256 + (size_t)n * (48 + 16) + (det ? (size_t)(2 * ch.turn_ints + 2) * sizeof(int) : 0);
  const bool can_one = max_pad <= QKF_XCAP_ONE / QK_TILE && (size_t)QKF_XCAP_ONE * 16 + lds_meta <= 160 * 1024;
  const bool can_two = max_pad <= QKF_XCAP_TWO / QK_TILE && (size_t)QKF_XCAP_TWO * 16 + lds_meta <= 160 * 1024 / QKF_TWO_WGS;
  const bool fused = p.variant == 20 && !f32 && !quad && p.fused_path != 0 && max_pad > (p.fused_path >= 2 ? 16 : 32) && (can_one || can_two);
  const bool second_class = fused && plan.n_first > 0 && plan.n_first < np;
  const bool split = second_class && can_one && can_two && p.fused_wgs == 0 && p.fused_split != 0 && !plan.second_wave2 && (p.fused_split == 2 || np >= 100ll * num_cus);
  const bool mixed = second_class && plan.second_wave2 && p.wave2_path && p.wave2_ring;
  const bool fused_two = fused && can_two && !split && (!can_one || p.fused_wgs == 2 || (p.fused_wgs == 0 && plan.fit_two >= 0.75 && plan.fit_narrow >= 0.5));
  const bool dual = fused && !fused_two && p.fused_dual;
  const int wgs = fused ? (fused_two ? QKF_TWO_WGS : 1) : p.wgs_per_cu;
  const long long grid = std::min(units, (long long)wgs * num_cus);
  ch.scratch_bytes = (size_t)(split ? 2ll * num_cus : grid) * (size_t)chains * 2 * (size_t)(ch.x_plane + ch.t_plane) * sizeof(double);
  const size_t site_meta = 16 + (size_t)(4 * (n + 1) + 2) * sizeof(int) + (size_t)2 * n * sizeof(long long);
  const size_t lds_ring = 3 * 16 * 1024 + site_meta;
  const size_t esz = f32 ? sizeof(float) : sizeof(double), lds_small = (size_t)(3 * 2 * (64 / esz) * 64 + 6 * 32 * 32) * esz + site_meta;
  if (lds_ring > 80 * 1024)
    return ch.rc = QK_EINVAL, snprintf(ch.err, sizeof ch.err, "qk_gram_values: %d sites need %zu bytes of LDS per workgroup (limit 80 KiB for 2 workgroups per CU)", n, lds_ring), ch;
  QkSweepRun& r = ch.run[0];
  ch.n_runs = 1, ch.launched_grid = r.grid = grid, r.count = np;
  if (quad) {
#ifdef QK_LAB
    r.kernel = QK_KERNEL_LAB;
#else
    ch.rc = QK_EINVAL, snprintf(ch.err, sizeof ch.err, "qk_gram_values: QK_PLAN_QUADS plans are swept by an experimental kernel that only libqklab.so contains");
#endif
  } else if (p.variant == 20 && p.wave_path && !f32 && max_pad <= 16) {
    r.kernel = QK_KERNEL_WAVE, ch.launched_grid = r.grid = std::min(np, 16ll * num_cus);
  } else if (!fused && p.variant == 20 && p.wave2_path && (!f32 || p.wave2_ring) && max_pad <= 32) {
    r.kernel = (f32 || p.wave2_ring) ? QK_KERNEL_WAVE2 : QK_KERNEL_WAVE2_PLAIN, ch.launched_grid = r.grid = std::min(np, 8ll * num_cus);
    ch.interleaved = ch.tails = true, ch.queues = plan.nq > 1 ? 8 : 1, r.nq = plan.nq;
  } else if (!fused && p.variant == 20 && p.small_path && max_pad <= 32 && lds_small <= 80 * 1024) {
    r.kernel = QK_KERNEL_SMALL, r.lds = lds_small;
  } else if (fused) {
    ch.interleaved = ch.fused_images = ch.tails = true, ch.queues = plan.nq > 1 ? 8 : 1, r.nq = plan.nq;
    r.kernel = fused_two ? (det ? QK_KERNEL_FUSED2_DET : QK_KERNEL_FUSED2) : dual ? (det ? QK_KERNEL_FUSED_DUAL_DET : QK_KERNEL_FUSED_DUAL) : (det ? QK_KERNEL_FUSED1_DET : QK_KERNEL_FUSED1);
    r.lds = (size_t)(fused_two ? QKF_XCAP_TWO : QKF_XCAP_ONE) * 16 + lds_meta;
    auto gang_of = [&](const long long g) { return p.gang && plan.nq > 1 && g >= 16 && g % 8 == 0 ? (int)(g / 8) : 0; };
    if (split || mixed) {
      QkSweepRun& r2 = ch.run[1];
      ch.n_runs = 2;
      r.count = plan.n_first, r2.first = plan.n_first, r2.count = np - plan.n_first;
      r.nq = r2.nq = plan.nq > 1 ? 8 : plan.nq;
      r.grid = std::min(r.count, (long long)wgs * num_cus);
      if (split) {
        r2.kernel = det ? QK_KERNEL_FUSED2_DET : QK_KERNEL_FUSED2, r2.grid = std::min(r2.count, (long long)QKF_TWO_WGS * num_cus);
        r2.lds = (size_t)QKF_XCAP_TWO * 16 + lds_meta, r2.gang_n = gang_of(r2.grid), r2.gang2 = true;
      } else {
        r2.kernel = QK_KERNEL_WAVE2, r2.grid = std::min(r2.count, 8ll * num_cus);
      }
    }
    r.gang_n = gang_of(r.grid);
  } else if (f32 || p.variant == 20) {
    r.kernel = QK_KERNEL_RING, r.lds = lds_ring;
  } else {
#ifdef QK_LAB
    r.kernel = QK_KERNEL_LAB;
#else
    ch.rc = QK_EINVAL, snprintf(ch.err, sizeof ch.err, "qk_gram_values: no kernel for this call");
#endif
  }
  return ch;
}
```

qml-cutensornet_amd/csrc/qkgram.hip:

```cpp
#include "qk_host.h"
#include "qk_ring.h"
#include "qk_fused.h"
#ifndef QKF_QUAD
#define QKF_QUAD 0
#endif
#if QKF_QUAD
#include "qk_quad.h"
#endif

#include <algorithm>
#include <cmath>
#include <cstdarg>
#include <cstdio>
#include <cstdlib>
#include <cstring>
#include <new>
#include <numeric>
#include <string>
#include <vector>

static thread_local std::string g_err;

int qk_fail(int code, const char* fmt, ...) {
  char buf[512];
// ... 26 lines not shown
    const char* e = std::getenv("QK_ROCTX");
    const char* pre = std::getenv("LD_PRELOAD");
    const bool attached = std::getenv("ROCP_TOOL_LIBRARIES") || (pre && std::strstr(pre, "rocprofiler"));
    if (e ? std::atoi(e) == 0 : !attached) return x;
    void* h = nullptr;
    for (const char* name : {"librocprofiler-sdk-roctx.so.1", "librocprofiler-sdk-roctx.so", "libroctx64.so.4", "libroctx64.so"})
      if ((h = dlopen(name, RTLD_NOW | RTLD_GLOBAL))) break;
    if (!h) return x;
    x.push = reinterpret_cast<int (*)(const char*)>(dlsym(h, "roctxRangePushA"));
    x.pop = reinterpret_cast<int (*)()>(dlsym(h, "roctxRangePop"));
    if (!x.push || !x.pop) x.push = nullptr, x.pop = nullptr;
    return x;
  }();
  return r;
}
}
extern "C" int qk_range_push(const char* name) {
  Roctx& r = roctx();
  return (r.push && name) ? r.push(name) : 0;
}
extern "C" int qk_range_pop(void) {
  Roctx& r = roctx();
  return r.pop ? r.pop() : 0;
}

static inline int pad16(int x) { return (x + TILE - 1) / TILE * TILE; }

extern "C" int64_t qk_pack_state_size(int32_t n_sites, const int32_t* bond_dims) {
  int64_t tot = 0;
  for (int k = 0; k < n_sites; ++k) tot += 2ll * pad16(bond_dims[k]) * 2 * pad16(bond_dims[k + 1]);
  return tot;
}

extern "C" int qk_pack_state(int32_t n_sites, const int32_t* bond_dims, const double* const* site_tensors,
                             int32_t layout, double* out, int64_t* site_offsets) {
  if (n_sites <= 0 || !bond_dims || !site_tensors || !out) return fail(QK_EINVAL, "qk_pack_state: null argument");
  if (layout != QK_LAYOUT_LPR && layout != QK_LAYOUT_LRP) return fail(QK_EINVAL, "qk_pack_state: unknown layout %d", layout);
  if (bond_dims[0] != 1 || bond_dims[n_sites] != 1) return fail(QK_EINVAL, "qk_pack_state: boundary bonds must be 1");
  int64_t off = 0;
  for (int k = 0; k < n_sites; ++k) {
    const int cl = bond_dims[k], cr = bond_dims[k + 1];
    if (cl <= 0 || cr <= 0) return fail(QK_EINVAL, "qk_pack_state: non-positive bond at site %d", k);
    const int pl = pad16(cl), pr = pad16(cr);
    const int64_t plane = (int64_t)pl * 2 * pr;
    double* re = out + off;
    double* im = re + plane;
    std::memset(re, 0, sizeof(double) * 2 * plane);
    const double* src = site_tensors[k];
    if (!src) return fail(QK_EINVAL, "qk_pack_state: null tensor at site %d", k);
    for (int l = 0; l < cl; ++l)
      for (int p = 0; p < 2; ++p)
        for (int r = 0; r < cr; ++r) {
          const int64_t s = (layout == QK_LAYOUT_LPR) ? (((int64_t)l * 2 + p) * cr + r) : (((int64_t)l * cr + r) * 2 + p);
          const int64_t d = ((int64_t)l * 2 + p) * pr + r;
          re[d] = src[2 * s];
          im[d] = src[2 * s + 1];
        }
    if (site_offsets) site_offsets[k] = off;
    off += 2 * plane;
  }
  return QK_OK;
}

#ifndef QKF_ONE_NW
#define QKF_ONE_NW 12
#define QKF_ONE_S 2
#define QKF_ONE_WPS 3
#endif
#ifndef QKF_TWO_NW
#define QKF_TWO_NW 8
#define QKF_TWO_S 1
#define QKF_TWO_WPS 4
#endif
#define QKF_KERNEL_ONE qk_sweep_fused_kernel<QKF_ONE_NW, QKF_ONE_S, QKF_XCAP_ONE, QKF_ONE_WPS>
#define QKF_KERNEL_TWO qk_sweep_fused_kernel<QKF_TWO_NW, QKF_TWO_S, QKF_XCAP_TWO, QKF_TWO_WPS>
#ifndef QKF_DUAL_NW
#define QKF_DUAL_NW 12
#define QKF_DUAL_WPS 3
#endif
#define QKF_KERNEL_DUAL qk_sweep_fused_dual_kernel<QKF_DUAL_NW, QKF_XCAP_ONE, QKF_DUAL_WPS>
#define QKF_KERNEL_ONE_DET qk_sweep_fused_kernel<QKF_ONE_NW, QKF_ONE_S, QKF_XCAP_ONE, QKF_ONE_WPS, true>
#define QKF_KERNEL_TWO_DET qk_sweep_fused_kernel<QKF_TWO_NW, QKF_TWO_S, QKF_XCAP_TWO, QKF_TWO_WPS, true>
#define QKF_KERNEL_DUAL_DET qk_sweep_fused_dual_kernel<QKF_DUAL_NW, QKF_XCAP_ONE, QKF_DUAL_WPS, true>
#if QKF_QUAD
#define QKF_QUAD_NW 8
#define QKF_KERNEL_QUAD qk_sweep_fused_quad_kernel<QKF_QUAD_NW, QKF_XCAP_ONE, 2>
#endif

extern "C" int qk_plan_destroy(qk_plan* plan) {
  if (!plan) return QK_OK;
  if (plan->d_pairs) (void)hipFree(plan->d_pairs);
  if (plan->d_groups) (void)hipFree(plan->d_groups);
  if (plan->d_seg) (void)hipFree(plan->d_seg);
  delete plan;
  return QK_OK;
}
__global__ void qk_convert_f32_kernel(const double* __restrict__ src, float* __restrict__ dst, const long long n) {
  for (long long e = (long long)blockIdx.x * blockDim.x + threadIdx.x; e < n; e += (long long)gridDim.x * blockDim.x) dst[e] = (float)src[e];
}

__global__ void qk_scatter_kernel(const int32_t* __restrict__ pairs, const double* __restrict__ vals, long long n,
                                  double* __restrict__ K, long long ld, int mirror) {
  const long long t = (long long)blockIdx.x * blockDim.x + threadIdx.x;
  if (t >= n) return;
  const int i = pairs[2 * t], j = pairs[2 * t + 1];
  if (i < 0) return;
  const double v = vals[t];
  K[(long long)j * ld + i] = v;
  if (mirror) K[(long long)i * ld + j] = v;
}

typedef double qk_v2d __attribute__((ext_vector_type(2)));

__device__ __forceinline__ void qk_ctile(QkfTile& t, const qk_v2d* __restrict__ P, const long pk, const long pm, const qk_v2d* __restrict__ Q, const long qk, const long qn, const int ks4,
                                         const int q, const int j) {
  const qk_v2d* pp = P + q * pk + j * pm;
  const qk_v2d* qq = Q + q * qk + j * qn;
  v4d p1 = {0, 0, 0, 0}, p2 = {0, 0, 0, 0}, p3 = {0, 0, 0, 0};
  qk_v2d a = pp[0], b = qq[0];
  for (int ks = 0; ks < ks4; ++ks) {
    const qk_v2d a0 = a, b0 = b;
    if (ks + 1 < ks4) a = pp[(long)4 * (ks + 1) * pk], b = qq[(long)4 * (ks + 1) * qk];
    qkf_kstep<false>(p1, p2, p3, a0.x, a0.y, b0.x, b0.y);
  }
  t.re = p1 - p2, t.im = p3 - p1 - p2;
}

__global__ __launch_bounds__(256) void qk_edge_kernel(const qk_v2d* __restrict__ il, const int32_t* __restrict__ dims, const int32_t* __restrict__ dtrue, const int64_t* __restrict__ offs,
                                                      const int n_sites, const int k, const long long n_states, qk_v2d* __restrict__ edge, const long long* __restrict__ edge_offs,
                                                      qk_v2d* __restrict__ tmp, const long long tmp_elems) {
  qk_v2d* const t0 = tmp + (long long)blockIdx.x * 2 * tmp_elems;
  qk_v2d* const t1 = t0 + tmp_elems;
  const int n1 = n_sites + 1, lane = threadIdx.x & 63, wave = threadIdx.x >> 6, nw = blockDim.x >> 6, j = lane & 15, q = lane >> 4;
  for (long long t = blockIdx.x; t < 2 * n_states; t += gridDim.x) {
    const long long st = t >> 1;
    const int right = (int)(t & 1);
    const int32_t* d = dims + st * n1;
    const int32_t* dt = dtrue + st * n1;
    qk_v2d* const dst = edge + edge_offs[t];
    for (int e = threadIdx.x; e < 256; e += blockDim.x) t0[e] = (qk_v2d){e == 0 ? 1.0 : 0.0, 0.0};
    __syncthreads();
    const qk_v2d* in = t0;
    for (int jj = 0; jj < k; ++jj) {
      const int site = right ? n_sites - 1 - jj : jj;
      const int lp = d[site], rp = d[site + 1];
      const qk_v2d* const A = il + (offs[st * n_sites + site] >> 1);
      const int ld_in = right ? rp : lp, ld_out = right ? lp : rp, rows_in = 1 << jj;
      const int ks4 = ((right ? dt[site + 1] : dt[site]) + 3) >> 2;
      qk_v2d* const out = (jj + 1 == k) ? dst : (in == t0 ? t1 : t0);
      const int nts = (rows_in + 15) >> 4, ntc = ld_out >> 4;
      for (int u = wave; u < nts * 2 * ntc; u += nw) {
        const int tc = u % ntc, pp = (u / ntc) & 1, ts = u / (2 * ntc);
        QkfTile T;
        if (right) qk_ctile(T, in + (long)(ts * 16) * ld_in, 1, ld_in, A + (long)pp * rp + (long)(tc * 16) * 2 * rp, 1, 2 * rp, ks4, q, j);
        else qk_ctile(T, in + (long)(ts * 16) * ld_in, 1, ld_in, A + (long)pp * rp + tc * 16, 2 * rp, 1, ks4, q, j);
#pragma unroll
        for (int r = 0; r < 4; ++r) {
          const int s_ = ts * 16 + q + 4 * r;
          if (s_ < rows_in) out[(long)(2 * s_ + pp) * ld_out + tc * 16 + j] = (qk_v2d){T.re[r], T.im[r]};
        }
      }
      __syncthreads();
      in = out;
    }
  }
}
// ... 43 lines not shown
      const v4d re = acc[c][0] - acc[c][1], im = acc[c][2] - acc[c][0] - acc[c][1];
#pragma unroll
      for (int r = 0; r < 4; ++r) dst[(long)(4 * (tl * 16 + q + 4 * r) + c) * rp + tr * 16 + j] = (qk_v2d){re[r], im[r]};
    }
  }
}

__global__ __launch_bounds__(256) void qk_segment_kernel(const int32_t* __restrict__ xdims, const int32_t* __restrict__ xtrue, const int32_t* __restrict__ ydims, const int32_t* __restrict__ ytrue,
                                                         const int n_sites, const int ek, const int32_t* __restrict__ pairs, const long long npairs, const QkSegRule rule, const int parities,
                                                         const bool greedy, const int assoc, const int switch_price, unsigned long long* __restrict__ seg) {
  const long long p = (long long)blockIdx.x * blockDim.x + threadIdx.x;
  if (p >= npairs) return;
  const long long xo = (long long)pairs[2 * p] * (n_sites + 1), yo = (long long)pairs[2 * p + 1] * (n_sites + 1);
  QkSegMask o{{0ull, 0ull}};
  const QkSegMask m = qk_segment_chain(xdims + xo, xtrue + xo, ydims + yo, ytrue + yo, n_sites, ek, rule, parities, greedy, nullptr, nullptr, assoc, switch_price, &o);
  seg[4 * p] = m.w[0], seg[4 * p + 1] = m.w[1], seg[4 * p + 2] = o.w[0], seg[4 * p + 3] = o.w[1];
}

#ifdef QK_LAB
__global__ void qk_lab_fold_kernel(const int64_t* __restrict__ src, int64_t* __restrict__ dst, const long long n, const long long win) {
  for (long long i = blockIdx.x * (long long)blockDim.x + threadIdx.x; i < n; i += (long long)gridDim.x * blockDim.x) dst[i] = (src[i] % win) & ~1ll;
}
#endif
__global__ void qk_selftest_f32_kernel(const float* __restrict__ P, const float* __restrict__ Q, float* __restrict__ C) {
  const int lane = threadIdx.x & 63, j = lane & 15, q = lane >> 4;
  v4f acc = {0, 0, 0, 0};
  for (int ks = 0; ks < 4; ++ks) acc = __builtin_amdgcn_mfma_f32_16x16x4f32(P[(4 * ks + q) * 16 + j], Q[(4 * ks + q) * 16 + j], acc, 0, 0, 0);
  for (int r = 0; r < 4; ++r) C[(4 * q + r) * 16 + j] = acc[r];
}

__global__ void qk_selftest_kernel(const double* __restrict__ P, const double* __restrict__ Q, double* __restrict__ C) {
  const int lane = threadIdx.x & 63, j = lane & 15, q = lane >> 4;
  v4d acc = {0, 0, 0, 0};
  for (int ks = 0; ks < 4; ++ks) acc = __builtin_amdgcn_mfma_f64_16x16x4f64(P[(4 * ks + q) * 16 + j], Q[(4 * ks + q) * 16 + j], acc, 0, 0, 0);
  for (int r = 0; r < 4; ++r) C[(q + 4 * r) * 16 + j] = acc[r];
}

extern "C" int qk_device_count(void) {
  int n = 0;
  if (hipGetDeviceCount(&n) != hipSuccess) return 0;
  return n;
}

static int ctx_init(qk_ctx* c, int device_id, int num_cus);

extern "C" int qk_ctx_create(int device_id, qk_ctx** out) {
  if (!out) return fail(QK_EINVAL, "qk_ctx_create: null out");
  int n = 0;
  hipError_t e = hipGetDeviceCount(&n);
  if (e != hipSuccess || n <= 0)
    return fail(QK_EDEVICE, "qk_ctx_create: no HIP device available (%s); this engine has no CPU fallback",
                e == hipSuccess ? "device count is 0" : hipGetErrorString(e));
  if (device_id < 0 || device_id >= n) return fail(QK_EINVAL, "qk_ctx_create: device %d out of range [0,%d)", device_id, n);
  HIP_TRY(hipSetDevice(device_id));
  hipDeviceProp_t prop;
  HIP_TRY(hipGetDeviceProperties(&prop, device_id));
  if (std::strncmp(prop.gcnArchName, "gfx950", 6) != 0)
    return fail(QK_EDEVICE, "qk_ctx_create: device %d is %s; this library is built for gfx950 only", device_id, prop.gcnArchName);
  qk_ctx* c = new (std::nothrow) qk_ctx;
  if (!c) return fail(QK_ENOMEM, "qk_ctx_create: out of memory");
  const int rc_init = ctx_init(c, device_id, prop.multiProcessorCount);
  if (rc_init != QK_OK) {
    qk_ctx_destroy(c);
    return rc_init;
  }
  *out = c;
  return QK_OK;
}

static int ctx_init(qk_ctx* c, int device_id, int num_cus) {
  c->device = device_id;
  c->num_cus = num_cus;
  HIP_TRY(hipStreamCreateWithFlags(&c->own_stream, hipStreamNonBlocking));
  c->stream = c->own_stream;
  HIP_TRY(hipEventCreate(&c->ev0));
  HIP_TRY(hipEventCreate(&c->ev1));
  HIP_TRY(hipEventCreate(&c->ev_mid));
  HIP_TRY(hipEventCreate(&c->ev_d));
  HIP_TRY(c->counter.alloc((QK_NQ_MAX * QK_QSTRIDE + 8 + 2 * 8 * QK_QSTRIDE) * sizeof(unsigned long long)));
  HIP_TRY(c->prof.alloc(8 * sizeof(unsigned long long)));
  HIP_TRY(hipMemset(c->prof.get(), 0, 8 * sizeof(unsigned long long)));
  for (const void* k : {(const void*)qk_sweep_ring_kernel<float>, (const void*)qk_sweep_ring_kernel<double>, (const void*)qk_sweep_small_kernel<double>, (const void*)qk_sweep_small_kernel<float>})
    HIP_TRY(hipFuncSetAttribute(k, hipFuncAttributeMaxDynamicSharedMemorySize, 80 * 1024));
  for (const void* k : {(const void*)QKF_KERNEL_ONE, (const void*)QKF_KERNEL_DUAL, (const void*)QKF_KERNEL_ONE_DET, (const void*)QKF_KERNEL_DUAL_DET})
    HIP_TRY(hipFuncSetAttribute(k, hipFuncAttributeMaxDynamicSharedMemorySize, 160 * 1024));
  for (const void* k : {(const void*)QKF_KERNEL_TWO, (const void*)QKF_KERNEL_TWO_DET}) HIP_TRY(hipFuncSetAttribute(k, hipFuncAttributeMaxDynamicSharedMemorySize, 160 * 1024 / QKF_TWO_WGS));
#if QKF_QUAD
  HIP_TRY(hipFuncSetAttribute(reinterpret_cast<const void*>(QKF_KERNEL_QUAD), hipFuncAttributeMaxDynamicSharedMemorySize, 160 * 1024));
#endif
  QkSweepPolicy& p = c->policy;
#ifdef QK_LAB
  {
    const int rc = qk_lab_init(c);
    if (rc != QK_OK) return rc;
  }
  if (const char* v = std::getenv("QK_VARIANT")) p.variant = std::atoi(v);
#endif
  if (const char* v = std::getenv("QK_SMALL")) p.small_path = std::atoi(v) != 0;
  if (const char* v = std::getenv("QK_WAVE")) p.wave_path = std::atoi(v) != 0;
  if (const char* v = std::getenv("QK_WAVE2")) p.wave2_path = std::atoi(v) != 0, p.wave2_ring = std::atoi(v) != 2;
  if (const char* v = std::getenv("QK_FUSED")) p.fused_path = std::atoi(v);
  if (const char* v = std::getenv("QK_MERGE")) p.merge_mode = std::max(0, std::min(2, std::atoi(v)));
  if (const char* v = std::getenv("QK_ASSOC")) p.assoc_mode = std::max(0, std::min(3, std::atoi(v)));
  if (const char* v = std::getenv("QK_SWITCH_PRICE")) p.switch_price = std::max(0, std::min(100000, std::atoi(v)));
  if (const char* v = std::getenv("QK_DETERMINISTIC"))
    if (std::atoi(v) != 0) p.deterministic = true, p.assoc_mode = 0;
  if (const char* v = std::getenv("QK_FUSED_SPLIT")) p.fused_split = std::max(0, std::min(2, std::atoi(v)));
  if (const char* v = std::getenv("QK_FUSED_WGS")) p.fused_wgs = std::max(0, std::min(2, std::atoi(v)));
  if (const char* v = std::getenv("QK_WGS_PER_CU")) p.wgs_per_cu = std::max(1, std::min(4, std::atoi(v)));
  return QK_OK;
}

extern "C" int qk_ctx_destroy(qk_ctx* c) {
  if (!c) return QK_OK;
  (void)hipSetDevice(c->device);
  if (c->stream) (void)hipStreamSynchronize(c->stream);
  if (c->ev0) (void)hipEventDestroy(c->ev0);
  if (c->ev1) (void)hipEventDestroy(c->ev1);
  if (c->ev_mid) (void)hipEventDestroy(c->ev_mid);
  if (c->ev_d) (void)hipEventDestroy(c->ev_d);
  if (c->own_stream) (void)hipStreamDestroy(c->own_stream);
  delete c;
  return QK_OK;
}

extern "C" int qk_ctx_trim(qk_ctx* c) {
  if (!c) return fail(QK_EINVAL, "qk_ctx_trim: null context");
  HIP_TRY(hipSetDevice(c->device));
  HIP_TRY(hipStreamSynchronize(c->stream));
  for (QkGrowBuf* b : {&c->scratch, &c->build_arena, &c->build_work, &c->derive_tmp, &c->local_scratch}) b->reset();
  return QK_OK;
}

extern "C" int qk_ctx_set_stream(qk_ctx* c, void* s) {
  if (!c) return fail(QK_EINVAL, "qk_ctx_set_stream: null context");
  c->stream = reinterpret_cast<hipStream_t>(s);
  return QK_OK;
}

extern "C" int qk_ctx_use_own_stream(qk_ctx* c) {
  if (!c) return fail(QK_EINVAL, "qk_ctx_use_own_stream: null context");
  c->stream = c->own_stream;
  return QK_OK;
}

extern "C" int qk_ctx_synchronize(qk_ctx* c) {
  if (!c) return fail(QK_EINVAL, "qk_ctx_synchronize: null context");
  HIP_TRY(hipSetDevice(c->device));
  HIP_TRY(hipStreamSynchronize(c->stream));
  return QK_OK;
}

int qk_mps_set_alloc(qk_ctx* c, int n_states, int n_sites, int64_t data_bytes, int precision, qk_mps_set** out, const char* who) {
  qk_mps_set* m = new (std::nothrow) qk_mps_set;
  if (!m) return fail(QK_ENOMEM, "%s: out of memory", who);
  m->ctx = c, m->n_states = n_states, m->n_sites = n_sites, m->precision = precision, m->bytes = data_bytes;
  const size_t nd = (size_t)n_states * (n_sites + 1), no = (size_t)n_states * n_sites;
  hipError_t e = m->d_data.alloc((size_t)data_bytes);
  if (e == hipSuccess) e = m->d_dims.alloc(nd * sizeof(int32_t));
  if (e == hipSuccess) e = m->d_true.alloc(nd * sizeof(int32_t));
  if (e == hipSuccess) e = m->d_offs.alloc(no * sizeof(int64_t));
  if (e != hipSuccess) {
    qk_mps_set_destroy(m);
    return fail(QK_EDEVICE, "%s: hipMalloc of a set of %lld bytes and its tables failed: %s", who, (long long)data_bytes, hipGetErrorString(e));
  }
  *out = m;
  return QK_OK;
// ... 292 lines not shown
    for (const qk_mps_set* m : {xs, ys})
      if ((rc = ensure_merged(c, const_cast<qk_mps_set*>(m), ek, merge_mode >= 2 ? 1 : 2)) != QK_OK) return rc;
    a.xmg = xs->d_mg.get<double>(), a.xmg_offs = xs->d_mg_offs.get<int64_t>(), a.ymg = ys->d_mg.get<double>(), a.ymg_offs = ys->d_mg_offs.get<int64_t>(), a.merge_steps = xs->mg_steps;
  }
#ifdef QK_LAB
  if (const char* v = std::getenv("QK_DEBUG_ALIAS")) {
    const long long win = std::atoll(v);
    if (win > 0) {
      auto fold = [&](const int64_t* src, const long long n) -> const int64_t* {
        QkDevBuf buf;
        if (buf.alloc((size_t)n * sizeof(int64_t)) != hipSuccess) return src;
        int64_t* dst = static_cast<int64_t*>(buf.release());
        qk_lab_fold_kernel<<<dim3(256), dim3(256), 0, c->stream>>>(src, dst, n, win);
        return dst;
      };
      a.xoffs = fold(a.xoffs, (long long)xs->n_states * xs->n_sites), a.yoffs = fold(a.yoffs, (long long)ys->n_states * ys->n_sites);
      if (a.merge_steps > 0)
        a.xmg_offs = fold(a.xmg_offs, (long long)xs->n_states * xs->mg_steps), a.ymg_offs = fold(a.ymg_offs, (long long)ys->n_states * ys->mg_steps);
    }
  }
#endif
  return QK_OK;
}

static QkSegRule seg_rule_of(const int kernel) {
  switch (kernel) {
    case QK_KERNEL_FUSED1: case QK_KERNEL_FUSED1_DET: return {QKF_XCAP_ONE, QKF_ONE_NW * QKF_ONE_S, false};
    case QK_KERNEL_FUSED2: case QK_KERNEL_FUSED2_DET: return {QKF_XCAP_TWO, QKF_TWO_NW * QKF_TWO_S, false};
#if QKF_QUAD
    case QK_KERNEL_FUSED_DUAL: return {QKF_XCAP_ONE, QKF_QUAD_NW, true};
#else
    case QK_KERNEL_FUSED_DUAL: return {QKF_XCAP_ONE, QKF_DUAL_NW, true};
#endif
    case QK_KERNEL_FUSED_DUAL_DET: return {QKF_XCAP_ONE, QKF_DUAL_NW, true};
    default: return {0, 0, false};
  }
}

static bool seg_assoc_of(const int kernel) {
#if QKF_QUAD
  if (kernel == QK_KERNEL_FUSED_DUAL) return false;
#endif
  return kernel == QK_KERNEL_FUSED_DUAL || kernel == QK_KERNEL_FUSED1 || kernel == QK_KERNEL_FUSED2;
}

static int ensure_segments(qk_ctx* c, const qk_mps_set* xs, const qk_mps_set* ys, qk_plan* plan, const QkSweepChoice& ch, const int merge_mode, SweepArgs& a) {
  const long long np = (long long)plan->pairs.size() / 2;
  const bool both = merge_mode >= 2 && xs->mg_stride == 1 && ys->mg_stride == 1;
  const int assoc = merge_mode >= 2 ? c->policy.assoc_mode : 0, switch_price = c->policy.switch_price;
  const unsigned long long key[8] = {2ull | ((unsigned long long)assoc << 8) | ((unsigned long long)switch_price << 16),
                                     xs->uid,
                                     ys->uid,
                                     (unsigned long long)a.edge_k,
                                     both ? 3ull : 1ull,
                                     merge_mode == 1 ? 1ull : 0ull,
                                     (unsigned long long)ch.run[0].kernel | ((unsigned long long)(ch.n_runs > 1 ? ch.run[1].kernel : 0) << 32),
                                     (unsigned long long)ch.run[0].count};
  if (plan->d_seg && std::equal(key, key + 8, plan->seg_key)) return a.seg = plan->d_seg, QK_OK;
  if (plan->d_seg) {
    HIP_TRY(hipStreamSynchronize(c->stream));
    (void)hipFree(plan->d_seg), plan->d_seg = nullptr;
  }
  QkDevBuf seg;
  HIP_TRY(seg.alloc((size_t)np * 4 * sizeof(unsigned long long)));
  unsigned long long* const d = seg.get<unsigned long long>();
  for (int i = 0; i < ch.n_runs; ++i) {
    const QkSweepRun& r = ch.run[i];
    const QkSegRule rule = seg_rule_of(r.kernel);
    if (r.count <= 0) continue;
    if (rule.cap == 0) {
      HIP_TRY(hipMemsetAsync(d + 4 * r.first, 0, (size_t)r.count * 4 * sizeof(unsigned long long), c->stream));
      continue;
    }
    qk_segment_kernel<<<dim3((unsigned)((r.count + 255) / 256)), dim3(256), 0, c->stream>>>(a.xdims, a.xtrue, a.ydims, a.ytrue, a.n_sites, a.edge_k, a.pairs + 2 * r.first, r.count, rule, both ? 3 : 1,
                                                                                            merge_mode == 1, seg_assoc_of(r.kernel) ? assoc : 0, switch_price, d + 4 * r.first);
  }
  HIP_TRY(hipGetLastError());
  plan->d_seg = static_cast<unsigned long long*>(seg.release());
  std::copy(key, key + 8, plan->seg_key);
  a.seg = plan->d_seg;
  return QK_OK;
}

static int launch_sweep(const int kernel, const bool f32, const long long grid_, const size_t lds, const hipStream_t s, const SweepArgs& a) {
  const dim3 grid((unsigned)grid_);
  switch (kernel) {
    case QK_KERNEL_WAVE: qk_sweep_wave_kernel<0><<<grid, dim3(64), lds, s>>>(a); break;
    case QK_KERNEL_WAVE2: if (f32) qk_sweep_wave2_kernel<3, float><<<grid, dim3(64), lds, s>>>(a); else qk_sweep_wave2_kernel<3, double><<<grid, dim3(64), lds, s>>>(a); break;
    case QK_KERNEL_WAVE2_PLAIN: qk_sweep_wave2_kernel<0, double><<<grid, dim3(64), lds, s>>>(a); break;
    case QK_KERNEL_SMALL: if (f32) qk_sweep_small_kernel<float><<<grid, dim3(512), lds, s>>>(a); else qk_sweep_small_kernel<double><<<grid, dim3(512), lds, s>>>(a); break;
    case QK_KERNEL_RING: if (f32) qk_sweep_ring_kernel<float><<<grid, dim3(512), lds, s>>>(a); else qk_sweep_ring_kernel<double><<<grid, dim3(512), lds, s>>>(a); break;
    case QK_KERNEL_FUSED1: QKF_KERNEL_ONE<<<grid, dim3(64 * QKF_ONE_NW), lds, s>>>(a); break;
    case QK_KERNEL_FUSED1_DET: QKF_KERNEL_ONE_DET<<<grid, dim3(64 * QKF_ONE_NW), lds, s>>>(a); break;
    case QK_KERNEL_FUSED2: QKF_KERNEL_TWO<<<grid, dim3(64 * QKF_TWO_NW), lds, s>>>(a); break;
    case QK_KERNEL_FUSED2_DET: QKF_KERNEL_TWO_DET<<<grid, dim3(64 * QKF_TWO_NW), lds, s>>>(a); break;
#if QKF_QUAD
    case QK_KERNEL_FUSED_DUAL: QKF_KERNEL_QUAD<<<grid, dim3(64 * QKF_QUAD_NW), lds, s>>>(a); break;
#else
    case QK_KERNEL_FUSED_DUAL: QKF_KERNEL_DUAL<<<grid, dim3(64 * QKF_DUAL_NW), lds, s>>>(a); break;
#endif
    case QK_KERNEL_FUSED_DUAL_DET: QKF_KERNEL_DUAL_DET<<<grid, dim3(64 * QKF_DUAL_NW), lds, s>>>(a); break;
    default: return fail(QK_EINVAL, "qk_gram_values: no kernel for this call");
  }
  return QK_OK;
}

extern "C" int qk_gram_values(qk_ctx* c, const qk_mps_set* xs, const qk_mps_set* ys, const qk_plan* plan_c, double* values_dev, double* z_dev) {
  if (!c || !xs || !plan_c || !values_dev) return fail(QK_EINVAL, "qk_gram_values: null argument");
  qk_plan* plan = const_cast<qk_plan*>(plan_c);
  if (!ys) ys = xs;
  if (xs->ctx != c || ys->ctx != c) return fail(QK_EINVAL, "qk_gram_values: sets belong to another context");
  if (xs->n_sites != ys->n_sites || xs->n_sites != plan->n_sites) return fail(QK_EINVAL, "qk_gram_values: site counts differ (%d, %d, plan %d)", xs->n_sites, ys->n_sites, plan->n_sites);
  if (plan->nx != xs->n_states || plan->ny != ys->n_states) return fail(QK_EINVAL, "qk_gram_values: plan is for %dx%d states, sets hold %dx%d", plan->nx, plan->ny, xs->n_states, ys->n_states);
  QkRangeGuard range_("qk:sweep");
  HIP_TRY(hipSetDevice(c->device));
  const long long np = (long long)plan->pairs.size() / 2;
  c->last = plan->stats;
  c->split_pending = c->tail_pending = false;
  c->last.max_bond = std::max(xs->max_pad, ys->max_pad);
  c->last.kernel_ms = 0, c->last.grid = 0, c->last.kernel = QK_KERNEL_NONE, c->last.precision = xs->precision;
  if (np == 0) return QK_OK;
  int rc = ensure_plan_uploaded(c, plan);
  if (rc != QK_OK) return rc;
  if (xs->precision != ys->precision) return fail(QK_EINVAL, "qk_gram_values: the two sets differ in precision (fp%d, fp%d)", xs->precision, ys->precision);
  const bool f32 = (xs->precision == 32);
  if (f32) c->last.bytes *= 0.5;

  QkSweepPolicy pol = c->policy;
  if (const char* v = std::getenv("QK_FUSED_DUAL")) pol.fused_dual = std::atoi(v) != 0;
  if (const char* v = std::getenv("QK_GANG")) pol.gang = std::atoi(v) != 0;
  const QkSweepChoice ch = qk_choose_sweep(pol, *plan, {xs->max_pad, xs->precision, xs->n_sites}, {ys->max_pad, ys->precision, ys->n_sites}, c->num_cus);
  if (ch.rc != QK_OK) return fail(ch.rc, "%s", ch.err);
  c->last.queues = ch.queues, c->last.tail_frac = c->last.second_tail_frac = 0;
  if (ch.scratch_bytes > c->scratch.bytes) HIP_TRY(hipStreamSynchronize(c->stream));
  HIP_TRY(c->scratch.ensure(ch.scratch_bytes));
  SweepArgs a{};
  a.xdata = xs->d_data.get<double>(), a.xdims = xs->d_dims.get<int32_t>(), a.xtrue = xs->d_true.get<int32_t>(), a.xoffs = xs->d_offs.get<int64_t>();
  a.ydata = ys->d_data.get<double>(), a.ydims = ys->d_dims.get<int32_t>(), a.ytrue = ys->d_true.get<int32_t>(), a.yoffs = ys->d_offs.get<int64_t>();
  a.n_sites = xs->n_sites;
  a.pairs = plan->d_pairs, a.npairs = np;
  a.groups = plan->d_groups, a.ngroups = (long long)plan->groups.size() / 2;
  a.values = values_dev, a.z = z_dev;
  a.scratch = c->scratch.get<double>(), a.x_plane = ch.x_plane, a.t_plane = ch.t_plane, a.turn_ints = ch.turn_ints;
  unsigned long long* const counter = c->counter.get<unsigned long long>();
  a.counter = counter, a.prof = c->prof.get<unsigned long long>();
  for (int s_ = 0; s_ <= QK_NQ_MAX; ++s_) a.qstart[s_] = plan->nq > 1 ? plan->qstart[s_] : (s_ == 0 ? 0 : np);
  a.tail = counter + QK_NQ_MAX * QK_QSTRIDE, a.err = a.tail + 7, a.gang = a.tail + 8;
#ifdef QK_LAB
  if (const char* v = std::getenv("QK_DEBUG_FLAGS")) a.debug_flags = std::atoi(v);
  if (const char* v = std::getenv("QK_PRIO")) a.prio_mode = std::atoi(v);
#endif
  HIP_TRY(hipEventRecord(c->ev_d, c->stream));
  HIP_TRY(hipMemsetAsync(counter, 0, (QK_NQ_MAX * QK_QSTRIDE + 8 + 2 * 8 * QK_QSTRIDE) * sizeof(unsigned long long), c->stream));
  HIP_TRY(hipMemsetAsync(a.tail, 0xFF, 4 * sizeof(unsigned long long), c->stream));
  if (ch.interleaved) {
    for (const qk_mps_set* m : {xs, ys})
      if ((rc = ensure_interleaved(c, const_cast<qk_mps_set*>(m))) != QK_OK) return rc;
    a.xdata = xs->d_il.get<double>(), a.ydata = ys->d_il.get<double>();
  }
  if (ch.fused_images && (rc = derive_fused_images(c, xs, ys, plan, pol.merge_mode, a)) != QK_OK) return rc;
  if (a.merge_steps > 0 && (rc = ensure_segments(c, xs, ys, plan, ch, pol.merge_mode, a)) != QK_OK) return rc;
  HIP_TRY(hipEventRecord(c->ev0, c->stream));
  for (int i = 0; i < ch.n_runs; ++i) {
    const QkSweepRun& r = ch.run[i];
    SweepArgs ar = a;
    ar.npairs = r.count, ar.nq = r.nq, ar.gang_n = r.gang_n;
    if (i == 1) {
      HIP_TRY(hipEventRecord(c->ev_mid, c->stream));
      ar.pairs = a.pairs + 2 * r.first, ar.values = a.values + r.first, ar.z = a.z ? a.z + 2 * r.first : nullptr, ar.seg = a.seg ? a.seg + 4 * r.first : nullptr;
      ar.counter = counter + 8 * QK_QSTRIDE, ar.tail = a.tail + 2;
      if (plan->nq > 1)
        for (int s_ = 0; s_ <= 8; ++s_) ar.qstart[s_] = plan->qstart[8 + s_] - r.first;
      if (r.gang2) ar.gang = a.gang + 8 * QK_QSTRIDE;
      c->last.second_pairs = plan->second.pairs, c->last.second_flops = plan->second.flops, c->last.second_padded_flops = plan->second.padded_flops;
      c->last.second_bytes = plan->second.bytes, c->last.second_kernel = r.kernel;
      c->split_pending = true;
    }
#ifdef QK_LAB
    if (r.kernel == QK_KERNEL_LAB) rc = plan->quad ? qk_lab_launch_quad(c, ar, (int)r.grid, xs->n_sites, f32) : qk_lab_launch(c, pol.variant, ar, (int)r.grid, xs->n_sites);
    else
#endif
      rc = launch_sweep(r.kernel, f32, r.grid, r.lds, c->stream, ar);
    if (rc != QK_OK) return rc;
  }
  HIP_TRY(hipGetLastError());
  HIP_TRY(hipEventRecord(c->ev1, c->stream));
  c->ev_pending = true;
  c->last.kernel = ch.run[0].kernel, c->last.grid = (int)ch.launched_grid;
  c->tail_pending = ch.tails;
  return QK_OK;
}

extern "C" int qk_gram_values_host(qk_ctx* c, const qk_mps_set* xs, const qk_mps_set* ys, const qk_plan* plan, double* values_host, double* z_host) {
  if (!c || !plan || !values_host) return fail(QK_EINVAL, "qk_gram_values_host: null argument");
  const int64_t np = qk_plan_num_pairs(plan);
  if (np == 0) return QK_OK;
  HIP_TRY(hipSetDevice(c->device));
  QkDevBuf vals, z;
  HIP_TRY(vals.alloc((size_t)np * sizeof(double)));
  if (z_host) HIP_TRY(z.alloc((size_t)np * 2 * sizeof(double)));
  const int rc = qk_gram_values(c, xs, ys, plan, vals.get<double>(), z.get<double>());
  if (rc != QK_OK) return rc;
  HIP_TRY(hipMemcpyAsync(values_host, vals.get(), (size_t)np * sizeof(double), hipMemcpyDeviceToHost, c->stream));
  if (z_host) HIP_TRY(hipMemcpyAsync(z_host, z.get(), (size_t)np * 2 * sizeof(double), hipMemcpyDeviceToHost, c->stream));
  HIP_TRY(hipStreamSynchronize(c->stream));
  return QK_OK;
}

extern "C" int qk_scatter(qk_ctx* c, const int32_t* pairs_dev, const double* values_dev, int64_t n, double* k_dev, int64_t ld, int32_t mirror) {
  if (!c || !pairs_dev || !values_dev || !k_dev) return fail(QK_EINVAL, "qk_scatter: null argument");
  if (n <= 0) return QK_OK;
  QkRangeGuard range_("qk:scatter");
  HIP_TRY(hipSetDevice(c->device));
  const int bs = 256;
  hipLaunchKernelGGL(qk_scatter_kernel, dim3((unsigned)((n + bs - 1) / bs)), dim3(bs), 0, c->stream, pairs_dev, values_dev, (long long)n, k_dev, (long long)ld, (int)mirror);
  HIP_TRY(hipGetLastError());
  return QK_OK;
}

extern "C" const char* qk_kernel_name(int32_t kernel, int32_t precision) {
  const bool f32 = precision == 32;
  switch (kernel) {
    case QK_KERNEL_WAVE: return "qk_sweep_wave_kernel<0>";
    case QK_KERNEL_SMALL: return f32 ? "qk_sweep_small_kernel<float>" : "qk_sweep_small_kernel<double>";
    case QK_KERNEL_FUSED1: return "qk_sweep_fused_kernel<12, 2, 8192, 3, false>";
    case QK_KERNEL_FUSED2: return "qk_sweep_fused_kernel<8, 1, 4608, 4, false>";
    case QK_KERNEL_FUSED1_DET: return "qk_sweep_fused_kernel<12, 2, 8192, 3, true>";
    case QK_KERNEL_FUSED2_DET: return "qk_sweep_fused_kernel<8, 1, 4608, 4, true>";
    case QK_KERNEL_FUSED_DUAL_DET: return "qk_sweep_fused_dual_kernel<12, 8192, 3, true>";
    case QK_KERNEL_RING: return f32 ? "qk_sweep_ring_kernel<float>" : "qk_sweep_ring_kernel<double>";
    case QK_KERNEL_WAVE2: return precision == 32 ? "qk_sweep_wave2_kernel<3, float>" : "qk_sweep_wave2_kernel<3, double>";
    case QK_KERNEL_WAVE2_PLAIN: return "qk_sweep_wave2_kernel<0, double>";
    case QK_KERNEL_FUSED_DUAL: return "qk_sweep_fused_dual_kernel<12, 8192, 3, false>";
    case QK_KERNEL_LAB: return "(lab kernel)";
    default: return "(none)";
  }
}
#ifndef QKF_EXPERIMENT
static_assert(QKF_ONE_NW == 12 && QKF_ONE_S == 2 && QKF_ONE_WPS == 3 && QKF_TWO_NW == 8 && QKF_TWO_S == 1 && QKF_TWO_WPS == 4 && QKF_XCAP_ONE == 8192 && QKF_XCAP_TWO == 4608,
              "qk_kernel_name spells the fused sweep's template arguments");
#endif

extern "C" int qk_get_stats(qk_ctx* c, qk_stats* out) {
  if (!c || !out) return fail(QK_EINVAL, "qk_get_stats: null argument");
  if (c->ev_pending) {
    HIP_TRY(hipSetDevice(c->device));
    HIP_TRY(hipEventSynchronize(c->ev1));
    float ms = 0;
    HIP_TRY(hipEventElapsedTime(&ms, c->ev0, c->ev1));
    c->last.kernel_ms = ms;
    HIP_TRY(hipEventElapsedTime(&ms, c->ev_d, c->ev0));
    c->last.derive_ms = ms;
    if (c->tail_pending) {
      unsigned long long t[8];
      HIP_TRY(hipMemcpy(t, c->counter.get<unsigned long long>() + QK_NQ_MAX * QK_QSTRIDE, sizeof t, hipMemcpyDeviceToHost));
      auto frac = [](const unsigned long long start, const unsigned long long first_exit, const unsigned long long last_exit) {
        return (last_exit > start && first_exit <= last_exit && first_exit >= start) ? (double)(last_exit - first_exit) / (double)(last_exit - start) : 0.0;
      };
      if (t[7] != 0) return fail(QK_EDEVICE, "qk_get_stats: the ordered accumulation of the last sweep ran out of patience (a bug: please report); its results are not valid");
      c->last.tail_frac = frac(t[0], t[1], t[4]);
      if (c->split_pending) c->last.second_tail_frac = frac(t[2], t[3], t[6]);
      c->tail_pending = false;
    }
    if (c->split_pending) {
      HIP_TRY(hipEventElapsedTime(&ms, c->ev_mid, c->ev1));
      c->last.second_ms = ms;
      c->split_pending = false;
    }
    c->ev_pending = false;
#ifdef QKF_PROF
// ... 121 lines not shown
```

qml-cutensornet_amd/engine.py:

```python
from __future__ import annotations

import ctypes as C
import os
import weakref
from contextlib import contextmanager

import numpy as np

from . import program as _program

_HERE = os.path.dirname(os.path.abspath(__file__))
LIB_PATH = os.path.join(_HERE, "libqkgram.so")

QK_LAYOUT_LPR, QK_LAYOUT_LRP = 0, 1
QK_PLAN_SYMMETRIC = 1
QK_PLAN_QUADS = 2
QK_PLAN_ORIENT = 4


class QkError(RuntimeError):
    pass


class QkStats(C.Structure):
    _fields_ = [
        ("pairs", C.c_int64),
        ("flops", C.c_double),
        ("padded_flops", C.c_double),
        ("bytes", C.c_double),
        ("kernel_ms", C.c_double),
        ("grid", C.c_int32),
        ("max_bond", C.c_int32),
        ("kernel", C.c_int32),
        ("precision", C.c_int32),
        ("second_pairs", C.c_int64),
        ("second_flops", C.c_double),
        ("second_padded_flops", C.c_double),
        ("second_bytes", C.c_double),
        ("second_ms", C.c_double),
        ("second_kernel", C.c_int32),
        ("queues", C.c_int32),
        ("tail_frac", C.c_double),
        ("second_tail_frac", C.c_double),
        ("derive_ms", C.c_double),
    ]

    def as_dict(self):
        return {k: getattr(self, k) for k, _ in self._fields_}


_lib = None

_P = C.c_void_p
_BUILD_ARGS = [_P, C.c_int32, C.c_int32, C.c_int32, _P, _P, _P, C.c_double, C.c_double, C.c_int32, C.c_uint32]
_SCAN_ARGS = [C.c_int32, _P, _P, C.c_int32]
_MATS_ARGS = [C.c_int32, _P, C.c_int32, _P]
_CHAN_ARGS = [C.c_int32, _P, _P, _P, _P, C.c_int32, C.c_uint64, _P, _P, C.c_uint32]
_CHAN2_ARGS = [C.c_int32, _P, _P]
_SIGNATURES = [
    ("qk_last_error", C.c_char_p, []),
    ("qk_device_count", C.c_int, []),
    ("qk_ctx_create", C.c_int, [C.c_int, C.POINTER(_P)]),
    ("qk_ctx_destroy", C.c_int, [_P]),
    ("qk_ctx_set_stream", C.c_int, [_P, _P]),
    ("qk_ctx_use_own_stream", C.c_int, [_P]),
    ("qk_ctx_synchronize", C.c_int, [_P]),
    ("qk_ctx_trim", C.c_int, [_P]),
    ("qk_mps_set_create", C.c_int, [_P, C.c_int32, C.c_int32, _P, _P, C.c_int32, C.POINTER(_P)]),
    ("qk_mps_set_destroy", C.c_int, [_P]),
    ("qk_mps_set_info", C.c_int, [_P, C.POINTER(C.c_int32), C.POINTER(C.c_int32), C.POINTER(C.c_int32), C.POINTER(C.c_int64)]),
    ("qk_mps_set_image", C.c_int, [_P, C.POINTER(C.c_int64), C.POINTER(_P), _P, _P]),
    ("qk_mps_set_copy_image", C.c_int, [_P, _P, C.c_int64]),
    ("qk_mps_set_from_packed", C.c_int, [_P, C.c_int32, C.c_int32, _P, _P, _P, C.c_int64, C.POINTER(_P)]),
    ("qk_mps_set_precision", C.c_int, [_P]),
    ("qk_mps_set_to_f32", C.c_int, [_P, _P, C.POINTER(_P)]),
    ("qk_mps_set_compress", C.c_int, [_P, _P, C.c_int32, C.c_double, C.c_double, C.POINTER(_P), _P, _P]),
    ("qk_pack_state_size", C.c_int64, [C.c_int32, _P]),
    ("qk_pack_state", C.c_int, [C.c_int32, _P, _P, C.c_int32, _P, _P]),
    ("qk_plan_create", C.c_int, [C.c_int32, C.c_int32, _P, C.c_int32, _P, C.c_uint32, C.c_int32, C.c_int32, C.c_int32, C.POINTER(_P)]),
    ("qk_plan_destroy", C.c_int, [_P]),
    ("qk_plan_num_pairs", C.c_int64, [_P]),
    ("qk_plan_total_pairs", C.c_int64, [_P]),
    ("qk_plan_max_pairs_per_rank", C.c_int64, [_P]),
    ("qk_plan_pairs", _P, [_P]),
    ("qk_plan_stats", C.c_int, [_P, C.POINTER(QkStats)]),
    ("qk_plan_first_run", C.c_int64, [_P]),
    ("qk_plan_queues", C.c_int, [_P, _P]),
    ("qk_plan_edge_sites", C.c_int32, [_P]),
    ("qk_plan_create_all", C.c_int, [C.c_int32, C.c_int32, _P, C.c_int32, _P, C.c_uint32, C.c_int32, _P]),
    ("qk_plan_cost", C.c_int, [_P, C.POINTER(C.c_double), C.POINTER(C.c_int32), C.POINTER(C.c_double)]),
    ("qk_gram_values", C.c_int, [_P, _P, _P, _P, _P, _P]),
    ("qk_gram_values_host", C.c_int, [_P, _P, _P, _P, _P, _P]),
    ("qk_scatter", C.c_int, [_P, _P, _P, C.c_int64, _P, C.c_int64, C.c_int32]),
    ("qk_gram_host", C.c_int, [_P, _P, _P, _P, C.c_int64]),
    ("qk_overlaps_host", C.c_int, [_P, _P, _P, _P]),
    ("qk_get_stats", C.c_int, [_P, C.POINTER(QkStats)]),
    ("qk_local_paulis_host", C.c_int, [_P, _P, _P, _P]),
    ("qk_projected_gram_host", C.c_int, [_P, C.c_int32, C.c_int32, _P, C.c_int32, _P, C.c_double, _P, C.c_int64]),
    ("qk_local_pair_paulis_host", C.c_int, [_P, _P, _P, _P, _P]),
    ("qk_projected_pair_gram_host", C.c_int, [_P, C.c_int32, C.c_int32, _P, C.c_int32, _P, C.c_double, _P, C.c_int64]),
    ("qk_local_pair_paulis_dist_host", C.c_int, [_P, _P, C.c_int32, _P, _P, _P]),
    ("qk_projected_pair_gram_dist_host", C.c_int, [_P, C.c_int32, C.c_int32, C.c_int32, _P, C.c_int32, _P, C.c_double, _P, C.c_int64]),
    ("qk_pauli_strings_host", C.c_int, [_P, _P, C.c_int32, _P, _P, _P]),
    ("qk_operator_strings_host", C.c_int, [_P, _P, C.c_int32, _P, C.c_int32, _P, _P, _P]),
    ("qk_mpo_expectations_host", C.c_int, [_P, _P, C.c_int32, _P, _P, _P, _P]),
    ("qk_mps_set_apply_mpo", C.c_int, [_P, _P, _P, _P, C.POINTER(_P)]),
    ("qk_feature_gram_host", C.c_int, [_P, C.c_int32, C.c_int32, _P, C.c_int32, _P, C.c_double, _P, C.c_int64]),
    ("qk_bond_purities_host", C.c_int, [_P, _P, _P, _P]),
    ("qk_bond_spectra_host", C.c_int, [_P, _P, C.c_int32, _P, _P]),
    ("qk_block_values_host", C.c_int, [_P, _P, _P, _P, C.c_int32, C.c_int32, _P, _P]),
    ("qk_block_self_host", C.c_int, [_P, _P, C.c_int32, C.c_int32, _P, _P, _P]),
    ("qk_window_rdms_host", C.c_int, [_P, _P, C.c_int32, C.c_int32, _P, _P, _P]),
    ("qk_sample_host", C.c_int, [_P, _P, C.c_int32, _P, C.c_uint64, C.c_int64, _P, _P]),
    ("qk_amplitudes_host", C.c_int, [_P, _P, C.c_int32, _P, C.c_int32, _P, _P, _P, _P, _P]),
    ("qk_shot_block_sums_host", C.c_int, [_P, C.c_int32, C.c_int32, C.c_int32, C.c_int32, _P, C.c_int32, _P, C.c_int64, _P, C.c_int32, C.c_int32, _P, _P, _P]),
    ("qk_shadow_hist_host", C.c_int, [_P, C.c_int32, C.c_int32, C.c_int32, _P, _P, C.c_int32, C.c_int32, C.c_int32, _P, _P, C.c_int32, C.c_int64, _P, _P, _P]),
    ("qk_shot_strings_host", C.c_int, [_P, C.c_int32, C.c_int32, C.c_int32, _P, _P, C.c_int32, C.c_int32, _P, _P, _P]),
    ("qk_kernel_name", C.c_char_p, [C.c_int32, C.c_int32]),
    ("qk_selftest_mfma", C.c_int, [_P]),
    ("qk_build_mps", C.c_int, _BUILD_ARGS + [C.POINTER(_P)]),
    ("qk_built_info", C.c_int, [_P, _P, _P, _P, C.POINTER(C.c_int64), C.POINTER(C.c_double)]),
    ("qk_built_launch", C.c_int, [_P, C.POINTER(C.c_int32), C.POINTER(C.c_int32), C.POINTER(C.c_int32)]),
    ("qk_built_download", C.c_int, [_P, _P]),
    ("qk_built_destroy", C.c_int, [_P]),
    ("qk_mps_set_from_built", C.c_int, [_P, _P, C.POINTER(_P)]),
    ("qk_build_program", C.c_int, [_P, _P, _P, C.POINTER(_P)]),
    ("qk_program_size", C.c_uint32, []),
# ... 2391 lines not shown
```

Before: 781,900.

## Keep more of the X environment resident in a larger LDS buffer with partial residency

Adds a larger LDS X buffer (RCAP, sized to nearly the whole 160 KiB LDS) for the one-wave-group and dual fused kernels. A per-site residency record built in the step table says which row tiles of X stay in LDS and which spill to global scratch. The old all-or-nothing global/LDS switch becomes a per-tile mask, and the side ping-pong buffer is now used for large sites too. The aim is to cut global scratch round trips for big bond dimensions, at the cost of more LDS per block (possibly lower occupancy) and more branching in the inner loop.

```diff
diff --git a/include/qkgram.h b/include/qkgram.h
--- a/include/qkgram.h
+++ b/include/qkgram.h
@@ -41,6 +41,7 @@
   int32_t queues;
   double tail_frac, second_tail_frac;
   double derive_ms;
+  int32_t lds_bytes, second_lds_bytes;
 } qk_stats;
 
 #define QK_KERNEL_NONE 0
diff --git a/lab/qk_quad.h b/lab/qk_quad.h
--- a/lab/qk_quad.h
+++ b/lab/qk_quad.h
@@ -197,7 +197,7 @@
     const v4i r0 = rec[3 * k], r1 = rec[3 * k + 1], r2 = rec[3 * k + 2];
     QkfSite s;
     s.a = rfl(r0.x), s.a2 = rfl(r0.y), s.b = rfl(r0.z), s.b2 = rfl(r0.w);
-    s.at = rfl(r1.x), s.nks = rfl(r1.y), s.W = rfl(r1.z), s.small = rfl(r1.w) != 0;
+    s.at = rfl(r1.x), s.nks = rfl(r1.y), s.W = rfl(r1.z), s.small = (rfl(r1.w) & QK_REC_SMALL) != 0;
     s.inv = rfl(r2.x);
     s.ps = rfl(r2.y), s.pd = 1 << s.ps, s.next = rfl(r2.z);
     s.mt = s.a / TILE, s.nt = s.b2 / TILE, s.nn = s.a2 / TILE;
diff --git a/qml-cutensornet_amd/csrc/qk_fused.h b/qml-cutensornet_amd/csrc/qk_fused.h
--- a/qml-cutensornet_amd/csrc/qk_fused.h
+++ b/qml-cutensornet_amd/csrc/qk_fused.h
@@ -1,6 +1,9 @@
 #pragma once
 #include "qk_device.h"
 #include "qk_plan.h"
+
+#include <cstddef>
+#include <type_traits>
 
 #define QKF_PRIO_LO() __builtin_amdgcn_s_setprio(0)
 #define QKF_PRIO_HI() __builtin_amdgcn_s_setprio(2)
@@ -587,6 +590,7 @@
 
 struct QkfSite {
   int a, a2, b, b2, at, nks, mt, nt, nn, W, inv, inv2, pd, ps, next;
+  int flags;
   bool small, sw;
   const v2d *Ak, *Bk;
 };
@@ -661,12 +665,13 @@
   *word = pp;
 }
 
-template <int NW, int S, int XCAP, int WPS, bool DET = false>
+template <int NW, int S, int XCAP, int WPS, bool DET = false, int RCAP = XCAP>
 __global__ __launch_bounds__(64 * NW, WPS) void qk_sweep_fused_kernel(const SweepArgs g) {
   constexpr int NT = 64 * NW;
   extern __shared__ __attribute__((aligned(16))) double lds_raw[];
   lds_v2d* const XL = (lds_v2d*)lds_raw;
-  long long* const slot = reinterpret_cast<long long*>(lds_raw + 2 * XCAP);
+  static_assert(RCAP >= XCAP && RCAP % QKF_XBLOCK == 0, "the buffer holds what the segmentation counts on, in whole blocks");
+  long long* const slot = reinterpret_cast<long long*>(lds_raw + 2 * RCAP);
   const v2d* const xdata = reinterpret_cast<const v2d*>(g.xdata);
   const v2d* const ydata = reinterpret_cast<const v2d*>(g.ydata);
   v2d* const G0 = reinterpret_cast<v2d*>(g.scratch) + (long long)blockIdx.x * 2 * g.x_plane;
@@ -690,7 +695,7 @@
     const v4i r0 = rec[3 * k], r1 = rec[3 * k + 1], r2 = rec[3 * k + 2];
     QkfSite s;
     s.a = rfl(r0.x), s.a2 = rfl(r0.y), s.b = rfl(r0.z), s.b2 = rfl(r0.w);
-    s.at = rfl(r1.x), s.nks = rfl(r1.y), s.W = rfl(r1.z), s.small = (rfl(r1.w) & QK_REC_SMALL) != 0, s.sw = (rfl(r1.w) & QK_REC_SWITCH) != 0;
+    s.at = rfl(r1.x), s.nks = rfl(r1.y), s.W = rfl(r1.z), s.flags = rfl(r1.w), s.small = (s.flags & QK_REC_SMALL) != 0, s.sw = (s.flags & QK_REC_SWITCH) != 0;
     s.inv = rfl(r2.x), s.inv2 = rfl(r2.w);
     s.ps = rfl(r2.y), s.pd = 1 << s.ps, s.next = rfl(r2.z);
     s.mt = s.a / TILE, s.nt = s.b2 / TILE, s.nn = s.a2 / TILE;
@@ -724,7 +729,7 @@
     __syncthreads();
     if (p < 0) break;
     const int xi = g.pairs[2 * p], yj = g.pairs[2 * p + 1];
-    qkf_step_table<XCAP, NT, true>(g, xi, yj, p, rec, m_off, tid, QkSegRule{XCAP, NW * S, false});
+    qkf_step_table<XCAP, NT, true>(g, xi, yj, p, rec, m_off, tid, QkSegRule{XCAP, NW * S, false, RCAP, QKF_RES_PARTIAL != 0});
     const int ek = g.edge_k, k_hi = ns - ek;
     const bool edges = ek > 0;
     if (!edges)
@@ -733,14 +738,12 @@
       for (int e = tid; e < 2 * g.turn_ints + 2; e += NT) tbroken[e] = 0;
     int tsel = 0;
     __syncthreads();
-    bool xg = false;
     int cur = 0, xb = 0;
     if (edges) {
       const v4i r0 = rec[3 * ek];
       const int a_e = rfl(r0.x), b_e = rfl(r0.z);
       const bool o1 = !DET && (rfl(rec[3 * ek + 1].w) & QK_REC_ORIENT) != 0;
-      xg = a_e * b_e > XCAP;
-      qkf_edge_prefix<NW, QKF_EDGE_PAIRS(WPS), QKF_EDGE_SETS(WPS)>(g, o1 ? yj : xi, o1 ? xi : yj, a_e, b_e, XL, G0, xg, wave, q, j, o1);
+      qkf_edge_prefix<NW, QKF_EDGE_PAIRS(WPS), QKF_EDGE_SETS(WPS)>(g, o1 ? yj : xi, o1 ? xi : yj, a_e, b_e, XL, G0, a_e * b_e > XCAP, wave, q, j, o1);
       __syncthreads();
     }
     QKF_STAMP(0);
@@ -756,18 +759,16 @@
       const bool small = sc.small;
       v2d* const Gc = G0 + (long long)cur * g.x_plane;
       v2d* const Gn = G0 + (long long)(cur ^ 1) * g.x_plane;
-      if (small && xg) {
-        for (int e = tid; e < a * b; e += NT) XL[e] = Gc[e];
+      const int n_out = sc.b2 * a2;
+      const QkResident rs = qk_rec_resident(sc.flags, mt, n_out, RCAP, xb != 0);
+      if (a * b <= XCAP && rs.khi - rs.klo < mt) {
+        const int e0 = (rs.klo == 0 ? rs.khi : 0) * (b * TILE), e1 = (rs.klo == 0 ? mt : rs.klo) * (b * TILE);
+        for (int e = e0 + tid; e < e1; e += NT) Gc[e] = XL[xb + e];
         __syncthreads();
-        xg = false, xb = 0;
-      } else if (!small && !xg) {
-        for (int e = tid; e < a * b; e += NT) Gc[e] = XL[xb + e];
-        __syncthreads();
-        xg = true;
-      }
-      const int n_out = sc.b2 * a2;
-      const bool pingpong = small && a * b + n_out <= XCAP;
-      const int ob = !small ? 0 : pingpong ? (xb == 0 ? XCAP - n_out : 0) : 0;
+      }
+      const unsigned xgm = qk_res_global_mask(rs);
+      const bool pingpong = rs.kind == QK_RES_SIDE;
+      const int ob = rs.ob;
       if (pingpong && !DET)
         for (int e = tid; e < n_out; e += NT) XL[ob + e] = (v2d){0.0, 0.0};
       QKF_STAMP(1);
@@ -776,8 +777,8 @@
         lds_int* const tcur = turn0 + tsel * g.turn_ints;
         if constexpr (DET) {
           for (int e = tid; e < g.turn_ints; e += NT) turn0[(tsel ^ 1) * g.turn_ints + e] = 0;
-        } else if (!small) {
-          for (int e = tid; e < w * TILE * a2; e += NT) XL[e] = (v2d){0.0, 0.0};
+        } else if (!small && !pingpong) {
+          for (int e = tid; e < w * TILE * a2; e += NT) XL[ob + e] = (v2d){0.0, 0.0};
           QKF_STEP_BARRIER();
         }
         QKF_STAMP(6);
@@ -794,15 +795,25 @@
                 const int ta = item_of(sc, w, it).ta;
                 const bool more = s + 1 < L && it + NW < items;
                 const QkfStream nxt = more ? b_stream(sc, s0, w, it + NW) : a_stream(sc, w, it0);
-                qkf_p1_tile(T[S - 1], fr, primed, b_stream(sc, s0, w, it), xbase, (unsigned)(ta * (b * TILE) + q * TILE + j), sc.nks, nxt);
+                const unsigned xoff = (unsigned)(ta * (b * TILE) + q * TILE + j);
+                if constexpr (std::is_same<decltype(xbase), std::nullptr_t>::value) {
+                  if ((xgm >> ta) & 1u) qkf_p1_tile(T[S - 1], fr, primed, b_stream(sc, s0, w, it), (const v2d*)Gc, xoff, sc.nks, nxt);
+                  else qkf_p1_tile(T[S - 1], fr, primed, b_stream(sc, s0, w, it), (const lds_v2d*)(XL + xb), xoff, sc.nks, nxt);
+                } else {
+                  qkf_p1_tile(T[S - 1], fr, primed, b_stream(sc, s0, w, it), xbase, xoff, sc.nks, nxt);
+                }
                 primed = true;
               }
             }
           };
-          if (xg) phase1((const v2d*)Gc);
-          else phase1((const lds_v2d*)(XL + xb));
+          if constexpr (S == 1) {
+            if (it0 < items && ((xgm >> item_of(sc, w, it0).ta) & 1u)) phase1((const v2d*)Gc);
+            else phase1((const lds_v2d*)(XL + xb));
+          } else {
+            phase1(nullptr);
+          }
           QKF_STAMP(2);
-          if (small && r0 == 0 && !(DET && pingpong)) {
+          if ((small || pingpong) && r0 == 0 && !(DET && pingpong)) {
             QKF_STEP_BARRIER();
             if (!pingpong && !DET) {
               for (int e = tid; e < n_out; e += NT) XL[e] = (v2d){0.0, 0.0};
@@ -846,19 +857,15 @@
           QKF_STAMP(1);
         }
       }
-      if (!small) {
-        if (nt > W) cur ^= 1;
-        else xg = false, xb = 0;
-      } else {
-        xb = ob;
-      }
+      if (nt > W) cur ^= 1, xb = 0;
+      else xb = ob;
     }
     const int fl_end = DET ? 0 : rfl(rec[3 * (k_hi - 1) + 1].w);
     const bool sw_end = (fl_end & QK_REC_SWITCH) != 0, o_end = ((fl_end & QK_REC_ORIENT) != 0) != sw_end;
     if (edges) {
       const v4i r0 = rec[3 * (k_hi - 1)];
       const int a_l = rfl(r0.y), b_l = rfl(r0.w), a_e = sw_end ? b_l : a_l, b_e = sw_end ? a_l : b_l;
-      qkf_edge_suffix<NW, QKF_EDGE_PAIRS(WPS), QKF_EDGE_SETS(WPS)>(g, o_end ? yj : xi, o_end ? xi : yj, a_e, b_e, (const lds_v2d*)(XL + xb), (const v2d*)(G0 + (long long)cur * g.x_plane), xg, zacc, wave,
+      qkf_edge_suffix<NW, QKF_EDGE_PAIRS(WPS), QKF_EDGE_SETS(WPS)>(g, o_end ? yj : xi, o_end ? xi : yj, a_e, b_e, (const lds_v2d*)(XL + xb), (const v2d*)(G0 + (long long)cur * g.x_plane), a_e * b_e > XCAP, zacc, wave,
                                                                    q, j, o_end);
       __syncthreads();
     }
@@ -866,7 +873,7 @@
       v2d zz = {0.0, 0.0};
       if (edges)
         for (int w_ = 0; w_ < NW; ++w_) zz.x += zacc[2 * w_], zz.y += zacc[2 * w_ + 1];
-      else zz = xg ? G0[(long long)cur * g.x_plane] : (v2d)XL[xb];
+      else zz = (v2d)XL[xb];
       if (o_end) zz.y = -zz.y;
       g.values[p] = zz.x * zz.x + zz.y * zz.y;
       if (g.z) {
@@ -1066,12 +1073,13 @@
   qkf_p2_block<FULL, HAS1>(t0, t1, s0, s1, fr, kmax, nxt.base, nxt.base + nxt.step, nxt.base + 2 * nxt.step, nxt.base + 3 * nxt.step, nxt.off, d, d1, rs);
 }
 
-template <int NW, int XCAP, int WPS, bool DET = false>
+template <int NW, int XCAP, int WPS, bool DET = false, int RCAP = XCAP>
 __global__ __launch_bounds__(64 * NW, WPS) void qk_sweep_fused_dual_kernel(const SweepArgs g) {
   constexpr int NT = 64 * NW;
   extern __shared__ __attribute__((aligned(16))) double lds_raw[];
   lds_v2d* const XL = (lds_v2d*)lds_raw;
-  long long* const slot = reinterpret_cast<long long*>(lds_raw + 2 * XCAP);
+  static_assert(RCAP >= XCAP && RCAP % QKF_XBLOCK == 0, "the buffer holds what the segmentation counts on, in whole blocks");
+  long long* const slot = reinterpret_cast<long long*>(lds_raw + 2 * RCAP);
   const v2d* const xdata = reinterpret_cast<const v2d*>(g.xdata);
   const v2d* const ydata = reinterpret_cast<const v2d*>(g.ydata);
   v2d* const G0 = reinterpret_cast<v2d*>(g.scratch) + (long long)blockIdx.x * 2 * g.x_plane;
@@ -1095,7 +1103,7 @@
     const v4i r0 = rec[3 * k], r1 = rec[3 * k + 1], r2 = rec[3 * k + 2];
     QkfSite s;
     s.a = rfl(r0.x), s.a2 = rfl(r0.y), s.b = rfl(r0.z), s.b2 = rfl(r0.w);
-    s.at = rfl(r1.x), s.nks = rfl(r1.y), s.W = rfl(r1.z), s.small = (rfl(r1.w) & QK_REC_SMALL) != 0, s.sw = (rfl(r1.w) & QK_REC_SWITCH) != 0;
+    s.at = rfl(r1.x), s.nks = rfl(r1.y), s.W = rfl(r1.z), s.flags = rfl(r1.w), s.small = (s.flags & QK_REC_SMALL) != 0, s.sw = (s.flags & QK_REC_SWITCH) != 0;
     s.inv = rfl(r2.x);
     s.ps = rfl(r2.y), s.pd = 1 << s.ps, s.next = rfl(r2.z);
     s.mt = s.a / TILE, s.nt = s.b2 / TILE, s.nn = s.a2 / TILE;
@@ -1139,7 +1147,7 @@
   auto table_of = [&](const long long pp) __attribute__((always_inline)) {
     if (pp < 0) return;
     const int xi_ = g.pairs[2 * pp], yj_ = g.pairs[2 * pp + 1];
-    qkf_step_table<XCAP, NT>(g, xi_, yj_, pp, rec, m_off, tid, QkSegRule{XCAP, NW, true});
+    qkf_step_table<XCAP, NT>(g, xi_, yj_, pp, rec, m_off, tid, QkSegRule{XCAP, NW, true, RCAP, QKF_RES_PARTIAL != 0});
   };
   table_of(p);
   while (p >= 0) {
@@ -1152,14 +1160,12 @@
       for (int e = tid; e < 2 * g.turn_ints + 2; e += NT) tbroken[e] = 0;
     int tsel = 0;
     __syncthreads();
-    bool xg = false;
     int cur = 0, xb = 0;
     if (edges) {
       const v4i r0 = rec[3 * ek];
       const int a_e = rfl(r0.x), b_e = rfl(r0.z);
       const bool o1 = !DET && (rfl(rec[3 * ek + 1].w) & QK_REC_ORIENT) != 0;
-      xg = a_e * b_e > XCAP;
-      qkf_edge_prefix<NW, QKF_EDGE_PAIRS(WPS), QKF_EDGE_SETS(WPS)>(g, o1 ? yj : xi, o1 ? xi : yj, a_e, b_e, XL, G0, xg, wave, q, j, o1);
+      qkf_edge_prefix<NW, QKF_EDGE_PAIRS(WPS), QKF_EDGE_SETS(WPS)>(g, o1 ? yj : xi, o1 ? xi : yj, a_e, b_e, XL, G0, a_e * b_e > XCAP, wave, q, j, o1);
       __syncthreads();
     }
     QKF_STAMP(0);
@@ -1175,18 +1181,16 @@
       const bool small = sc.small;
       v2d* const Gc = G0 + (long long)cur * g.x_plane;
       v2d* const Gn = G0 + (long long)(cur ^ 1) * g.x_plane;
-      if (small && xg) {
-        for (int e = tid; e < a * b; e += NT) XL[e] = Gc[e];
+      const int n_out = sc.b2 * a2;
+      const QkResident rs = qk_rec_resident(sc.flags, mt, n_out, RCAP, xb != 0);
+      if (a * b <= XCAP && rs.khi - rs.klo < mt) {
+        const int e0 = (rs.klo == 0 ? rs.khi : 0) * (b * TILE), e1 = (rs.klo == 0 ? mt : rs.klo) * (b * TILE);
+        for (int e = e0 + tid; e < e1; e += NT) Gc[e] = XL[xb + e];
         __syncthreads();
-        xg = false, xb = 0;
-      } else if (!small && !xg) {
-        for (int e = tid; e < a * b; e += NT) Gc[e] = XL[xb + e];
-        __syncthreads();
-        xg = true;
-      }
-      const int n_out = sc.b2 * a2;
-      const bool pingpong = small && a * b + n_out <= XCAP;
-      const int ob = !small ? 0 : pingpong ? (xb == 0 ? XCAP - n_out : 0) : 0;
+      }
+      const unsigned xgm = qk_res_global_mask(rs);
+      const bool pingpong = rs.kind == QK_RES_SIDE;
+      const int ob = rs.ob;
       if (pingpong && !DET)
         for (int e = tid; e < n_out; e += NT) XL[ob + e] = (v2d){0.0, 0.0};
       QKF_STAMP(1);
@@ -1195,8 +1199,8 @@
         lds_int* const tcur = turn0 + tsel * g.turn_ints;
         if constexpr (DET) {
           for (int e = tid; e < g.turn_ints; e += NT) turn0[(tsel ^ 1) * g.turn_ints + e] = 0;
-        } else if (!small) {
-          for (int e = tid; e < w * TILE * a2; e += NT) XL[e] = (v2d){0.0, 0.0};
+        } else if (!small && !pingpong) {
+          for (int e = tid; e < w * TILE * a2; e += NT) XL[ob + e] = (v2d){0.0, 0.0};
           QKF_STEP_BARRIER();
         }
         for (int r0 = 0; r0 < units; r0 += NW) {
@@ -1208,7 +1212,7 @@
           if (mine) {
             const QkfStream bs = b_stream(sc, s0, v, un.half), as = a_stream(sc, v);
             const unsigned xoff = (unsigned)(ta * (b * TILE) + q * TILE + j);
-            if (xg) {
+            if ((xgm >> ta) & 1u) {
               if (has1) qkf_p1_dual<true>(T0, T1, fr, fs, primed, bs, (const v2d*)Gc, xoff, sc.nks, as);
               else qkf_p1_dual<false>(T0, T1, fr, fs, primed, bs, (const v2d*)Gc, xoff, sc.nks, as);
             } else {
@@ -1217,7 +1221,7 @@
             }
           }
           QKF_STAMP(2);
-          if (small && r0 == 0 && !(DET && pingpong)) {
+          if ((small || pingpong) && r0 == 0 && !(DET && pingpong)) {
             QKF_STEP_BARRIER();
             if (!pingpong && !DET) {
               for (int e = tid; e < n_out; e += NT) XL[e] = (v2d){0.0, 0.0};
@@ -1274,12 +1278,8 @@
           __syncthreads();
         }
       }
-      if (!small) {
-        if (nt > W) cur ^= 1;
-        else xg = false, xb = 0;
-      } else {
-        xb = ob;
-      }
+      if (nt > W) cur ^= 1, xb = 0;
+      else xb = ob;
     }
     if (tid == QKF_PULLER(NT)) qkf_pull_next(g, xcc, gang_round, slot + (psel ^ 1));
     const int fl_end = DET ? 0 : rfl(rec[3 * (k_hi - 1) + 1].w);
@@ -1287,7 +1287,7 @@
     if (edges) {
       const v4i r0 = rec[3 * (k_hi - 1)];
       const int a_l = rfl(r0.y), b_l = rfl(r0.w), a_e = sw_end ? b_l : a_l, b_e = sw_end ? a_l : b_l;
-      qkf_edge_suffix<NW, QKF_EDGE_PAIRS(WPS), QKF_EDGE_SETS(WPS)>(g, o_end ? yj : xi, o_end ? xi : yj, a_e, b_e, (const lds_v2d*)(XL + xb), (const v2d*)(G0 + (long long)cur * g.x_plane), xg, zacc, wave,
+      qkf_edge_suffix<NW, QKF_EDGE_PAIRS(WPS), QKF_EDGE_SETS(WPS)>(g, o_end ? yj : xi, o_end ? xi : yj, a_e, b_e, (const lds_v2d*)(XL + xb), (const v2d*)(G0 + (long long)cur * g.x_plane), a_e * b_e > XCAP, zacc, wave,
                                                                    q, j, o_end);
     }
     __syncthreads();
@@ -1296,7 +1296,7 @@
       v2d zz = {0.0, 0.0};
       if (edges)
         for (int w_ = 0; w_ < NW; ++w_) zz.x += zacc[2 * w_], zz.y += zacc[2 * w_ + 1];
-      else zz = xg ? G0[(long long)cur * g.x_plane] : (v2d)XL[xb];
+      else zz = (v2d)XL[xb];
       if (o_end) zz.y = -zz.y;
       g.values[p] = zz.x * zz.x + zz.y * zz.y;
       if (g.z) {
diff --git a/qml-cutensornet_amd/csrc/qk_plan.h b/qml-cutensornet_amd/csrc/qk_plan.h
--- a/qml-cutensornet_amd/csrc/qk_plan.h
+++ b/qml-cutensornet_amd/csrc/qk_plan.h
@@ -19,6 +19,16 @@
 #endif
 static constexpr int QKF_XCAP_ONE = QKF_XCAP_ONE_V, QKF_XCAP_TWO = QKF_XCAP_TWO_V;
 static constexpr int QK_TILE = 16;
+#ifndef QKF_RES_PARTIAL
+#define QKF_RES_PARTIAL 1
+#endif
+#ifndef QKF_RES_BIG
+#define QKF_RES_BIG 1
+#endif
+static constexpr int QKF_LDS_BYTES = 160 * 1024, QKF_META_ROOM = 8 * 1024;
+static constexpr int QKF_RCAP_ONE = QKF_RES_BIG ? (QKF_LDS_BYTES - QKF_META_ROOM) / 16 / (QK_TILE * QK_TILE) * (QK_TILE * QK_TILE) : QKF_XCAP_ONE;
+static_assert(QKF_RCAP_ONE >= QKF_XCAP_ONE && (long long)QKF_RCAP_ONE * 16 + QKF_META_ROOM <= QKF_LDS_BYTES && QKF_RCAP_ONE % (QK_TILE * QK_TILE) == 0,
+              "the large X buffer and the room behind it fit the LDS of a CU; the buffer holds whole 16 x 16 blocks");
 static inline int qk_pad16(int x) { return (x + QK_TILE - 1) / QK_TILE * QK_TILE; }
 static constexpr int GMAX = 4;
 
@@ -68,6 +78,8 @@
 struct QkSegRule {
   int xcap, cap;
   bool dual;
+  int rcap = 0;
+  bool partial = false;
 };
 struct QkSegMask {
   unsigned long long w[2];
@@ -76,6 +88,38 @@
 QK_HD static inline bool qk_seg_one_round(const QkSegRule& r, const int pmt, const int nt) { return pmt * (r.dual ? (nt + 1) / 2 : nt) <= r.cap; }
 QK_HD static inline bool qk_seg_small(const QkSegRule& r, const int a, const int a2, const int b, const int b2, const int pd) {
   return a * b <= r.xcap && a2 * b2 <= r.xcap && (qk_seg_one_round(r, pd * (a / QK_TILE), b2 / QK_TILE) || a * b + a2 * b2 <= r.xcap);
+}
+static constexpr int QK_RES_NONE = 0, QK_RES_SIDE = 1, QK_RES_PART = 2, QK_RES_INPLACE = 3;
+struct QkResident {
+  int kind, ob;
+  int klo, khi;
+};
+QK_HD static inline int qk_res_cap(const QkSegRule& r) { return r.rcap > r.xcap ? r.rcap : r.xcap; }
+QK_HD static inline unsigned qk_res_global_mask(const QkResident& s) { return ~(unsigned)(((1ull << s.khi) - 1ull) & ~((1ull << s.klo) - 1ull)); }
+QK_HD static inline QkResident qk_resident(const QkSegRule& r, const int a, const int a2, const int b, const int b2, const int pd, const bool x_top) {
+  const int rcap = qk_res_cap(r), n_in = a * b, n_out = a2 * b2, mt = a / QK_TILE, panel = b * QK_TILE;
+  if (n_in > r.xcap || n_out > r.xcap) return QkResident{QK_RES_NONE, 0, 0, 0};
+  const int ob = x_top ? 0 : rcap - n_out;
+  if (n_in + n_out <= rcap) return QkResident{QK_RES_SIDE, ob, 0, mt};
+  if (qk_seg_small(r, a, a2, b, b2, pd)) return QkResident{QK_RES_INPLACE, 0, 0, mt};
+  if (!r.partial) return QkResident{QK_RES_NONE, 0, 0, 0};
+  if (x_top) {
+    const int over = n_out - (rcap - n_in), t0 = (over + panel - 1) / panel;
+    return QkResident{QK_RES_PART, ob, t0 < mt ? t0 : mt, mt};
+  }
+  const int t0 = ob / panel;
+  return QkResident{QK_RES_PART, ob, 0, t0 < mt ? t0 : mt};
+}
+static constexpr int QK_REC_KIND_SHIFT = 3, QK_REC_T0_LOW_SHIFT = 8, QK_REC_T0_TOP_SHIFT = 16;
+QK_HD static inline int qk_rec_resident_bits(const QkSegRule& r, const int a, const int a2, const int b, const int b2, const int pd) {
+  const QkResident lo = qk_resident(r, a, a2, b, b2, pd, false), hi = qk_resident(r, a, a2, b, b2, pd, true);
+  return (lo.kind << QK_REC_KIND_SHIFT) | (lo.khi << QK_REC_T0_LOW_SHIFT) | (hi.klo << QK_REC_T0_TOP_SHIFT);
+}
+QK_HD static inline QkResident qk_rec_resident(const int word, const int mt, const int n_out, const int rcap, const bool x_top) {
+  const int kind = (word >> QK_REC_KIND_SHIFT) & 3, t0 = (word >> (x_top ? QK_REC_T0_TOP_SHIFT : QK_REC_T0_LOW_SHIFT)) & 63;
+  const bool other_end = kind == QK_RES_SIDE || kind == QK_RES_PART;
+  if (kind == QK_RES_NONE) return QkResident{QK_RES_NONE, 0, 0, 0};
+  return QkResident{kind, other_end && !x_top ? rcap - n_out : 0, x_top ? t0 : 0, x_top ? mt : t0};
 }
 QK_HD static inline long long qk_step_instr(const int pd, const int a, const int a2, const int b, const int b2, const int at, const int bt) {
   return 3ll * pd * (b2 / QK_TILE) * ((long long)(a / QK_TILE) * ((bt + 3) >> 2) + (long long)(a2 / QK_TILE) * ((at + 3) >> 2));
@@ -187,7 +231,8 @@
   const bool small = qk_seg_small(rule, a, a2, b, b2, 2 * len);
   const int mt = a / QK_TILE, nt = b2 / QK_TILE;
   const int lim = rule.xcap / (QK_TILE * a2), W = small ? nt : (lim < 1 ? 1 : lim < nt ? lim : nt);
-  return QkStepRec{{a, a2, b, b2, xt[e], (yt[e] + 3) >> 2, W, (small ? QK_REC_SMALL : 0) | (o ? QK_REC_ORIENT : 0) | (sw ? QK_REC_SWITCH : 0), qk_recip20(mt), len == 2 ? 2 : 1, e + len,
+  return QkStepRec{{a, a2, b, b2, xt[e], (yt[e] + 3) >> 2, W, (small ? QK_REC_SMALL : 0) | (o ? QK_REC_ORIENT : 0) | (sw ? QK_REC_SWITCH : 0) | qk_rec_resident_bits(rule, a, a2, b, b2, 2 * len), qk_recip20(mt),
+                    len == 2 ? 2 : 1, e + len,
                     item_recips ? qk_unit_recips(nt, W, false) : 0}};
 }
 
@@ -237,6 +282,7 @@
   int switch_price = QK_SWITCH_PRICE;
   bool fused_dual = true;
   bool gang = false;
+  bool fused_big = true;
 };
 
 struct QkSetShape {
@@ -249,6 +295,8 @@
   size_t lds = 0;
   long long first = 0, count = 0;
   int nq = 1, gang_n = 0;
+  bool big = false;
+  size_t lds_launch = 0;
   bool gang2 = false;
 };
 
@@ -313,6 +361,8 @@
     ch.interleaved = ch.fused_images = ch.tails = true, ch.queues = plan.nq > 1 ? 8 : 1, r.nq = plan.nq;
     r.kernel = fused_two ? (det ? QK_KERNEL_FUSED2_DET : QK_KERNEL_FUSED2) : dual ? (det ? QK_KERNEL_FUSED_DUAL_DET : QK_KERNEL_FUSED_DUAL) : (det ? QK_KERNEL_FUSED1_DET : QK_KERNEL_FUSED1);
     r.lds = (size_t)(fused_two ? QKF_XCAP_TWO : QKF_XCAP_ONE) * 16 + lds_meta;
+    r.big = !fused_two && p.fused_big && QKF_RCAP_ONE > QKF_XCAP_ONE && lds_meta <= (size_t)QKF_META_ROOM;
+    if (r.big) r.lds_launch = (size_t)QKF_RCAP_ONE * 16 + lds_meta;
     auto gang_of = [&](const long long g) { return p.gang && plan.nq > 1 && g >= 16 && g % 8 == 0 ? (int)(g / 8) : 0; };
     if (split || mixed) {
       QkSweepRun& r2 = ch.run[1];
@@ -337,5 +387,7 @@
     ch.rc = QK_EINVAL, snprintf(ch.err, sizeof ch.err, "qk_gram_values: no kernel for this call");
 #endif
   }
+  for (int i = 0; i < ch.n_runs; ++i)
+    if (!ch.run[i].big) ch.run[i].lds_launch = ch.run[i].lds;
   return ch;
 }
diff --git a/qml-cutensornet_amd/csrc/qkgram.hip b/qml-cutensornet_amd/csrc/qkgram.hip
--- a/qml-cutensornet_amd/csrc/qkgram.hip
+++ b/qml-cutensornet_amd/csrc/qkgram.hip
@@ -132,6 +132,10 @@
 #define QKF_KERNEL_ONE_DET qk_sweep_fused_kernel<QKF_ONE_NW, QKF_ONE_S, QKF_XCAP_ONE, QKF_ONE_WPS, true>
 #define QKF_KERNEL_TWO_DET qk_sweep_fused_kernel<QKF_TWO_NW, QKF_TWO_S, QKF_XCAP_TWO, QKF_TWO_WPS, true>
 #define QKF_KERNEL_DUAL_DET qk_sweep_fused_dual_kernel<QKF_DUAL_NW, QKF_XCAP_ONE, QKF_DUAL_WPS, true>
+#define QKF_KERNEL_ONE_BIG qk_sweep_fused_kernel<QKF_ONE_NW, QKF_ONE_S, QKF_XCAP_ONE, QKF_ONE_WPS, false, QKF_RCAP_ONE>
+#define QKF_KERNEL_DUAL_BIG qk_sweep_fused_dual_kernel<QKF_DUAL_NW, QKF_XCAP_ONE, QKF_DUAL_WPS, false, QKF_RCAP_ONE>
+#define QKF_KERNEL_ONE_DET_BIG qk_sweep_fused_kernel<QKF_ONE_NW, QKF_ONE_S, QKF_XCAP_ONE, QKF_ONE_WPS, true, QKF_RCAP_ONE>
+#define QKF_KERNEL_DUAL_DET_BIG qk_sweep_fused_dual_kernel<QKF_DUAL_NW, QKF_XCAP_ONE, QKF_DUAL_WPS, true, QKF_RCAP_ONE>
 #if QKF_QUAD
 #define QKF_QUAD_NW 8
 #define QKF_KERNEL_QUAD qk_sweep_fused_quad_kernel<QKF_QUAD_NW, QKF_XCAP_ONE, 2>
@@ -341,7 +345,8 @@
   HIP_TRY(hipMemset(c->prof.get(), 0, 8 * sizeof(unsigned long long)));
   for (const void* k : {(const void*)qk_sweep_ring_kernel<float>, (const void*)qk_sweep_ring_kernel<double>, (const void*)qk_sweep_small_kernel<double>, (const void*)qk_sweep_small_kernel<float>})
     HIP_TRY(hipFuncSetAttribute(k, hipFuncAttributeMaxDynamicSharedMemorySize, 80 * 1024));
-  for (const void* k : {(const void*)QKF_KERNEL_ONE, (const void*)QKF_KERNEL_DUAL, (const void*)QKF_KERNEL_ONE_DET, (const void*)QKF_KERNEL_DUAL_DET})
+  for (const void* k : {(const void*)QKF_KERNEL_ONE, (const void*)QKF_KERNEL_DUAL, (const void*)QKF_KERNEL_ONE_DET, (const void*)QKF_KERNEL_DUAL_DET, (const void*)QKF_KERNEL_ONE_BIG,
+                        (const void*)QKF_KERNEL_DUAL_BIG, (const void*)QKF_KERNEL_ONE_DET_BIG, (const void*)QKF_KERNEL_DUAL_DET_BIG})
     HIP_TRY(hipFuncSetAttribute(k, hipFuncAttributeMaxDynamicSharedMemorySize, 160 * 1024));
   for (const void* k : {(const void*)QKF_KERNEL_TWO, (const void*)QKF_KERNEL_TWO_DET}) HIP_TRY(hipFuncSetAttribute(k, hipFuncAttributeMaxDynamicSharedMemorySize, 160 * 1024 / QKF_TWO_WGS));
 #if QKF_QUAD
@@ -800,8 +805,20 @@
   return QK_OK;
 }
 
-static int launch_sweep(const int kernel, const bool f32, const long long grid_, const size_t lds, const hipStream_t s, const SweepArgs& a) {
+static int launch_sweep(const int kernel, const bool f32, const long long grid_, const size_t lds, const hipStream_t s, const SweepArgs& a, const bool big) {
   const dim3 grid((unsigned)grid_);
+  if (big) {
+    const size_t lds_big = lds;
+    switch (kernel) {
+      case QK_KERNEL_FUSED1: QKF_KERNEL_ONE_BIG<<<grid, dim3(64 * QKF_ONE_NW), lds_big, s>>>(a); return QK_OK;
+      case QK_KERNEL_FUSED1_DET: QKF_KERNEL_ONE_DET_BIG<<<grid, dim3(64 * QKF_ONE_NW), lds_big, s>>>(a); return QK_OK;
+#if !QKF_QUAD
+      case QK_KERNEL_FUSED_DUAL: QKF_KERNEL_DUAL_BIG<<<grid, dim3(64 * QKF_DUAL_NW), lds_big, s>>>(a); return QK_OK;
+#endif
+      case QK_KERNEL_FUSED_DUAL_DET: QKF_KERNEL_DUAL_DET_BIG<<<grid, dim3(64 * QKF_DUAL_NW), lds_big, s>>>(a); return QK_OK;
+      default: return fail(QK_EINVAL, "qk_gram_values: kernel %d has no instantiation with the large X buffer", kernel);
+    }
+  }
   switch (kernel) {
     case QK_KERNEL_WAVE: qk_sweep_wave_kernel<0><<<grid, dim3(64), lds, s>>>(a); break;
     case QK_KERNEL_WAVE2: if (f32) qk_sweep_wave2_kernel<3, float><<<grid, dim3(64), lds, s>>>(a); else qk_sweep_wave2_kernel<3, double><<<grid, dim3(64), lds, s>>>(a); break;
@@ -846,6 +863,7 @@
 
   QkSweepPolicy pol = c->policy;
   if (const char* v = std::getenv("QK_FUSED_DUAL")) pol.fused_dual = std::atoi(v) != 0;
+  if (const char* v = std::getenv("QK_FUSED_BIG")) pol.fused_big = std::atoi(v) != 0;
   if (const char* v = std::getenv("QK_GANG")) pol.gang = std::atoi(v) != 0;
   const QkSweepChoice ch = qk_choose_sweep(pol, *plan, {xs->max_pad, xs->precision, xs->n_sites}, {ys->max_pad, ys->precision, ys->n_sites}, c->num_cus);
   if (ch.rc != QK_OK) return fail(ch.rc, "%s", ch.err);
@@ -898,12 +916,13 @@
     if (r.kernel == QK_KERNEL_LAB) rc = plan->quad ? qk_lab_launch_quad(c, ar, (int)r.grid, xs->n_sites, f32) : qk_lab_launch(c, pol.variant, ar, (int)r.grid, xs->n_sites);
     else
 #endif
-      rc = launch_sweep(r.kernel, f32, r.grid, r.lds, c->stream, ar);
+      rc = launch_sweep(r.kernel, f32, r.grid, r.lds_launch, c->stream, ar, r.big);
     if (rc != QK_OK) return rc;
   }
   HIP_TRY(hipGetLastError());
   HIP_TRY(hipEventRecord(c->ev1, c->stream));
   c->ev_pending = true;
+  c->last.lds_bytes = (int32_t)ch.run[0].lds_launch, c->last.second_lds_bytes = ch.n_runs > 1 ? (int32_t)ch.run[1].lds_launch : 0;
   c->last.kernel = ch.run[0].kernel, c->last.grid = (int)ch.launched_grid;
   c->tail_pending = ch.tails;
   return QK_OK;
diff --git a/qml-cutensornet_amd/engine.py b/qml-cutensornet_amd/engine.py
--- a/qml-cutensornet_amd/engine.py
+++ b/qml-cutensornet_amd/engine.py
@@ -43,6 +43,8 @@
         ("tail_frac", C.c_double),
         ("second_tail_frac", C.c_double),
         ("derive_ms", C.c_double),
+        ("lds_bytes", C.c_int32),
+        ("second_lds_bytes", C.c_int32),
     ]
 
     def as_dict(self):
```

Result: faster. 791,900 (median of 6 runs) (+1.3%).
